# XinMing0411/AC-VAE

Measured on AMD Instinct MI355X. Metric: train-step captions/s (and audio-sec/s) at B=32, 1/2/4/8 MI355X, higher is better.
Workload: dtype f32

## Files before the change

### acvae_amd/build.py

```python
import os
import subprocess
import sys
from concurrent.futures import ThreadPoolExecutor

HERE = os.path.dirname(os.path.abspath(__file__))
CSRC = os.path.join(HERE, "csrc")
LIB = os.path.join(HERE, "libacvae_hip.so")
HIPCC = os.environ.get("HIPCC", "/opt/rocm/bin/hipcc")
FLAGS = ["-O3", "--offload-arch=gfx950", "-fPIC", "-std=c++17", "-Wall", "-Wno-unused-function",
         "-ffp-contract=off"]
if os.environ.get("ACVAE_EXACT_TANH") == "1":
    FLAGS.append("-DACVAE_EXACT_TANH")


def sources():
    return sorted(f for f in os.listdir(CSRC) if f.endswith(".hip"))


def _newer(a, b):
    return (not os.path.exists(b)) or os.path.getmtime(a) > os.path.getmtime(b)


def parse_usage(text):
    import re
    out, name = {}, None
    for line in text.splitlines():
        m = re.search(r"Function Name: (\S+)", line)
        if m:
            name = m.group(1)
            out[name] = {}
            continue
        for key, pat in (("vgprs", r" VGPRs: (\d+)"), ("sgprs", r" SGPRs: (\d+)"), ("scratch", r"ScratchSize \[bytes/lane\]: (\d+)"),
                         ("occupancy", r"Occupancy \[waves/SIMD\]: (\d+)")):
            m = re.search(pat, line)
            if m and name:
                out[name][key] = int(m.group(1))
    return out


def resource_usage():
    usage = {}
    for s in sources():
        path = os.path.join(CSRC, s[:-4] + ".usage.txt")
        if os.path.exists(path):
            usage.update(parse_usage(open(path).read()))
    return usage


def build(force=False, verbose=False):
    hdrs = [os.path.join(CSRC, f) for f in os.listdir(CSRC) if f.endswith(".h")]
    hdrs.append(os.path.join(os.path.dirname(HERE), "include", "acvae_hip.h"))
    objs, jobs = [], []
    for s in sources():
        src = os.path.join(CSRC, s)
        obj = os.path.join(CSRC, s[:-4] + ".o")
        objs.append(obj)
        if force or _newer(src, obj) or any(_newer(h, obj) for h in hdrs) or not os.path.exists(obj[:-2] + ".usage.txt"):
            jobs.append([HIPCC, *FLAGS, "-Rpass-analysis=kernel-resource-usage", "-c", src, "-o", obj])

    def run(cmd):
        if verbose:
            print(" ".join(cmd), flush=True)
        r = subprocess.run(cmd, capture_output=True, text=True)
        if r.returncode != 0:
            raise RuntimeError("hipcc failed:\n" + " ".join(cmd) + "\n" + r.stdout + r.stderr)
        if "-c" in cmd:
            remarks = "\n".join(l for l in r.stderr.splitlines() if "kernel-resource-usage" in l)
            open(cmd[-1][:-2] + ".usage.txt", "w").write(remarks)
            import re as _re
            rest = "\n".join(l for l in r.stderr.splitlines() if "kernel-resource-usage" not in l and
                             not _re.match(r"^\s*(\d+)?\s*\|", l)).strip()
            if verbose:
                for k, u in sorted(parse_usage(remarks).items()):
                    if u.get("scratch", 0) or u.get("vgprs", 0) >= 200:
                        print(f"  {k[:90]}: {u.get('vgprs')} VGPRs, {u.get('scratch')} B/lane scratch, occupancy {u.get('occupancy')}")
                if rest:
                    print(rest)
        elif verbose and r.stderr.strip():
            print(r.stderr)

    with ThreadPoolExecutor(max_workers=min(6, max(1, len(jobs)))) as ex:
        list(ex.map(run, jobs))
    if jobs or not os.path.exists(LIB):
        run([HIPCC, "--offload-arch=gfx950", "-shared", "-fPIC", "-o", LIB, *objs])
    return LIB


if __name__ == "__main__":
    print(build(force="--force" in sys.argv, verbose=True))
```

### acvae_amd/csrc/conv.h

```cpp
#pragma once
#include <hip/hip_runtime.h>
#include <stdint.h>
#include "common.h"
#include "job_table.h"

struct DropoutSpec {
  float p;
  const uint8_t* mask;
  uint64_t seed;
  uint32_t site;
};

enum { UP_PLAIN = 0, UP_POOL = 1, UP_DROP = 2 };

namespace acvae {
int conv3x3_igemm(const float* X, const float* scale, const float* shift, const float* Wp, float* Y, float* partials,
                  int N, int H, int W, int Cin, int Cout, hipStream_t st);
int conv_partials_rows(int N, int H, int W);
int conv3x3_igemm_bf16(const bf16_t* X, const float* scale, const float* shift, const bf16_t* Wp, bf16_t* Y,
                       float* partials, int N, int H, int W, int Cin, int Cout, hipStream_t st);
long conv3x3_wgrad_bf16_slab_floats(int N, int H, int W, int Cin, int Cout);
int conv3x3_wgrad_bf16_splits(int N, int H, int W, int Cin, int Cout);
int conv3x3_wgrad_bf16_launch(const bf16_t* dY, const bf16_t* X, const float* scale, const float* shift, float* slab, int N,
                              int H, int W, int Cin, int Cout, hipStream_t st);
int wgrad_reduce(const float* slab, int nsplit, float* dW_oihw, int Cout, int Cin, hipStream_t st);
long conv3x3_wgrad_slab_floats(int N, int H, int W, int Cin, int Cout);
int conv3x3_wgrad(const float* dY, const float* X, const float* scale, const float* shift, float* dW_oihw, float* slab,
                  int N, int H, int W, int Cin, int Cout, hipStream_t st);
bool conv3x3_wino_ok(int H, int W, int Cin, int Cout);
long conv3x3_wino_weight_floats(int Cin, int Cout);
int conv_wino_partials_rows(int N, int H, int W);
int conv3x3_wino_weights(const float* W_oihw, float* U, int Cout, int Cin, bool dgrad, hipStream_t st);
struct WinoWeightsJob { const float* W; float* U; int Cout, Cin, dgrad; };
using WinoWeightsBatch = RangeTable<WinoWeightsJob, 32>;
int conv3x3_wino_weights_batch(WinoWeightsBatch& b, hipStream_t st);
struct WinoBnReduce { const float* Y; const float* scale; const float* shift; const float* mean; const float* invstd; };
int conv3x3_wino(const float* X, const float* scale, const float* shift, const float* U, float* Y, float* partials, int N,
                 int H, int W, int Cin, int Cout, hipStream_t st, const WinoBnReduce* red = nullptr);
bool conv3x3_wino_wgrad_ok(int H, int W, int Cin, int Cout);
long conv3x3_wino_wgrad_slab_floats(int N, int H, int W, int Cin, int Cout);
int conv3x3_wino_wgrad(const float* dY, const float* X, const float* scale, const float* shift, float* dW_oihw, float* slab,
                       int N, int H, int W, int Cin, int Cout, hipStream_t st);
template <class T>
int repack_weights(const float* W_oihw, T* Wf, T* Wd, int Cout, int Cin, hipStream_t st);
struct RepackJob { const float* W; void* dst; int Cout, Cin, dgrad; };
using RepackBatch = RangeTable<RepackJob, 32>;
template <class T>
int repack_weights_batch(RepackBatch& b, hipStream_t st);
inline int conv3x3_igemm(const bf16_t* X, const float* scale, const float* shift, const bf16_t* Wp, bf16_t* Y,
                         float* partials, int N, int H, int W, int Cin, int Cout, hipStream_t st) {
  return conv3x3_igemm_bf16(X, scale, shift, Wp, Y, partials, N, H, W, Cin, Cout, st);
}
inline int conv3x3_wgrad(const bf16_t* dY, const bf16_t* X, const float* scale, const float* shift, float* dW_oihw,
                         float* slab, int N, int H, int W, int Cin, int Cout, hipStream_t st) {
  int r = conv3x3_wgrad_bf16_launch(dY, X, scale, shift, slab, N, H, W, Cin, Cout, st);
  if (r != 0) return r;
  return wgrad_reduce(slab, conv3x3_wgrad_bf16_splits(N, H, W, Cin, Cout), dW_oihw, Cout, Cin, st);
}
template <class T>
inline long conv3x3_wgrad_slab_floats_t(int N, int H, int W, int Cin, int Cout) {
  return sizeof(T) == 2 ? conv3x3_wgrad_bf16_slab_floats(N, H, W, Cin, Cout) : conv3x3_wgrad_slab_floats(N, H, W, Cin, Cout);
}
int bn0_stats(const float* x, float* partials, long rows, int F, int* nparts, hipStream_t st);
int bn0_partials_rows(long rows);
int bn_finalize(const float* partials, int P, int C, double count, const float* gamma, const float* beta,
                float* running_mean, float* running_var, int64_t* nbt, int training, float* scale, float* shift,
                float* mean, float* invstd, double* dpart, hipStream_t st);
long colsum_scratch_doubles(int width);
int colsum_tickets_reset(double* dpart, hipStream_t st);
long colsum_ticket_words();
int colsum2(const float* x, int P, int width, double* dpart, float* out, float* out2, int split, hipStream_t st);
struct ColsumJob { const float* x; int P, width; float* out; float* out_b; int R; long d0; };
using ColsumBatch = RangeTable<ColsumJob, 6, int>;
int colsum_batch(ColsumBatch& b, double* dpart, long dpart_doubles, hipStream_t st);
int conv1_first_blocks(int N, int T);
template <class TY>
int conv1_first_fwd(const float* x, const float* scale0, const float* shift0, const float* W1, TY* Y,
                    float* partials, int N, int T, int F, hipStream_t st);
template <class TY>
int conv1_first_bwd(const float* x, const float* scale0, const float* shift0, const float* mean0, const float* invstd0,
                    const float* W1, const TY* dY, float* dw_part, float* bn_part, float* dW1, float* dgamma0,
                    float* dbeta0, double* dpart, int N, int T, int F, hipStream_t st);
template <class T>
int bn_relu_pool(const T* Y, const float* scale, const float* shift, T* P, int N, int H, int W, int C,
                 DropoutSpec drop, hipStream_t st, bool pool = true);
int bn_bwd_blocks(int N, int H, int W, int C);
template <class T>
int bn_bwd(const T* Y, const T* dO, int upstream, const float* scale, const float* shift, const float* mean,
           const float* invstd, float* partials, float* sum_g, float* sum_gy, T* dY, double* dpart, int N, int H,
           int W, int C, DropoutSpec drop, hipStream_t st, bool batch_stats = true, int ready_rows = 0);
template <class T>
int relu_mask(const T* Y, const float* scale, const float* shift, uint8_t* out, int N, int H, int W, int C, hipStream_t st);
template <class T>
int freq_mean(const T* P, float* out, long rows, int Fp, int C, hipStream_t st);
template <class T>
int freq_mean_bwd(const float* dae, T* dP, long rows, int Fp, int C, hipStream_t st);
int time_pool(const float* ae, float* out, int N, int S, int C, DropoutSpec drop, hipStream_t st);
int relu_dropout(float* x, int total, DropoutSpec drop, hipStream_t st);
}

int acvae_gemm_nt_dual(const float* A1, int64_t lda1, const float* B1, int64_t ldb1, int K1, const float* A2,
                       int64_t lda2, const float* B2, int64_t ldb2, int K2, const float* bias, float* C, int64_t ldc,
                       int M, int N, int accumulate, hipStream_t st, float* skws = nullptr);
int acvae_gemm_nt_pair(const float* A0, int64_t lda0, const float* B0, int64_t ldb0, int K0, const float* bias0, float* C0,
                       int64_t ldc0, int N0, int acc0, const float* A1, int64_t lda1, const float* B1, int64_t ldb1, int K1,
                       const float* bias1, float* C1, int64_t ldc1, int N1, int acc1, int M, hipStream_t st);
constexpr int TN_TICKETS = 256;
int acvae_gemm_tn_fused(const float* A, int64_t lda, const float* B, int64_t ldb, float* C, int64_t ldc, int M, int N, int K,
                        int accumulate, float* ws, int64_t ws_bytes, hipStream_t st);
long acvae_skinny_ws_floats();
long acvae_skinny_ticket_words();
int acvae_skinny_ws_reset(float* ws, hipStream_t st);
struct TransposeJob { const float* in; long ld_in; float* out; long ld_out; int rows, cols; };
using TransposeBatch = acvae::RangeTable<TransposeJob, 12, int>;
int acvae_transpose_batch(TransposeBatch& b, hipStream_t st);
```

### acvae_amd/csrc/decoder.hip

```cpp
#include <cstdlib>
#include "common.h"
#include "conv.h"
#include "rnn.h"
#include "decode_persist.h"
#include "../../include/acvae_hip.h"

namespace {

struct Bump {
  long off = 0;
  long take(long n) { const long o = off; off = (off + n + 63) & ~63L; return o; }
};

struct Ctx {
  hipStream_t s;
  float* skws;
  operator hipStream_t() const { return s; }
};
inline int gemm(const float* A, long lda, const float* B, long ldb, const float* bias, float* C, long ldc, int M, int N,
                int K, int acc, const Ctx& st) {
  return acvae_gemm_nt_dual(A, lda, B, ldb, K, nullptr, 0, nullptr, 0, 0, bias, C, ldc, M, N, acc, st.s, st.skws);
}
inline int gemm2(const float* A1, long lda1, const float* B1, long ldb1, int K1, const float* A2, long lda2,
                 const float* B2, long ldb2, int K2, const float* bias, float* C, long ldc, int M, int N, int acc,
                 const Ctx& st) {
  if (M <= 64)
    return acvae_gemm_nt_dual(A1, lda1, B1, ldb1, K1, A2, lda2, B2, ldb2, K2, bias, C, ldc, M, N, acc, st.s, st.skws);
  ACVAE_TRY(acvae_gemm_nt_dual(A1, lda1, B1, ldb1, K1, nullptr, 0, nullptr, 0, 0, bias, C, ldc, M, N, acc, st.s, st.skws));
  return acvae_gemm_nt_dual(A2, lda2, B2, ldb2, K2, nullptr, 0, nullptr, 0, 0, nullptr, C, ldc, M, N, 1, st.s, st.skws);
}
struct TnWs { float* p; long bytes; };
inline int gemm_tn(const float* A, long lda, const float* B, long ldb, float* C, long ldc, int M, int N, int K, TnWs ws,
                   hipStream_t st) {
  return acvae_gemm_tn_fused(A, lda, B, ldb, C, ldc, M, N, K, 0, ws.p, ws.bytes, st);
}
inline void zb_skinny(acvae::ZeroBatch& zb, float* skws) { zb.add(skws, acvae_skinny_ticket_words()); }
inline void zb_colsum(acvae::ZeroBatch& zb, double* dpart) { zb.add(dpart, acvae::colsum_ticket_words()); }
inline void zb_tn(acvae::ZeroBatch& zb, TnWs ws) { zb.add(ws.p, TN_TICKETS); }
inline int transp(const float* in, long ld_in, float* out, long ld_out, int rows, int cols, hipStream_t st) {
  return acvae_transpose(in, ld_in, out, ld_out, rows, cols, st);
}
inline int zero(float* p, long n, hipStream_t st) {
  return hipMemsetAsync(p, 0, (size_t)n * sizeof(float), st) == hipSuccess ? ACVAE_OK : (int)hipGetLastError();
}
struct Fork {
  hipStream_t main_s, aux;
  bool on() const { return aux != main_s; }
  static int edge(hipStream_t from, hipStream_t to) {
    constexpr int RING = 64;
    struct Ring { hipEvent_t ev[RING]; int next; int dev; };
    static thread_local Ring ring = {{}, 0, -1};
    int dev = -1;
    if (hipGetDevice(&dev) != hipSuccess) return (int)hipGetLastError();
    if (dev != ring.dev) {
      for (int i = 0; i < RING; ++i) ring.ev[i] = nullptr;
      ring.next = 0; ring.dev = dev;
    }
    hipEvent_t& e = ring.ev[ring.next];
    ring.next = (ring.next + 1) % RING;
    if (!e && hipEventCreateWithFlags(&e, hipEventDisableTiming) != hipSuccess) return (int)hipGetLastError();
    hipError_t r = hipEventRecord(e, from);
    if (r == hipSuccess) r = hipStreamWaitEvent(to, e, 0);
    return r == hipSuccess ? ACVAE_OK : (int)r;
  }
  int begin() const { return on() ? edge(main_s, aux) : ACVAE_OK; }
  int join() const { return on() ? edge(aux, main_s) : ACVAE_OK; }
};
inline long tn_ws_floats(int M, int N, int K) { return acvae_gemm_tn_workspace_bytes(M, N, K) / 4 + 64 + TN_TICKETS; }

enum {
  TP_DEC_EMB, TP_DEC_WIH, TP_DEC_WHH, TP_DEC_BIH, TP_DEC_BHH, TP_DEC_CLS_W, TP_DEC_CLS_B, TP_DEC_ATT_V, TP_DEC_ATT_W,
  TP_DEC_ATT_B, TP_Q_EMB, TP_Q_WIH, TP_Q_WHH, TP_Q_BIH, TP_Q_BHH, TP_Q_WIH_R, TP_Q_WHH_R, TP_Q_BIH_R, TP_Q_BHH_R,
  TP_Q_TML_W, TP_Q_TML_B, TP_P_EMB, TP_P_ATT_V, TP_P_ATT_W, TP_P_ATT_B, TP_P_WIH, TP_P_WHH, TP_P_BIH, TP_P_BHH,
  TP_P_ML_W, TP_P_ML_B, TP_MLO_W, TP_MLO_B, TP_LN_W, TP_LN_B, TP_COUNT
};
static_assert(TP_COUNT == ACVAE_TEXT_NPARAMS, "text parameter table out of sync with the header");

struct PostLayout {
  long words, x, hidden, save_f, save_r, hprev_f, hprev_r, argmax, saved_total;
  long gi_f, gi_r, gh, hf, ml, dml, dhid, dgi_f, dgi_r, dgh_f, dgh_r, dh_a, dh_b, dx, wt, wt2, wt_ih0, wt_ih1, wt_ml, pq_hbuf, pq_cnt, tn, dpart, skws,
       scratch_total;
  long tn_floats, dpart_doubles;
};
int post_layout(int N, int Tc, int E, int Hq, int V, PostLayout& L) {
  if (N <= 0 || Tc <= 0 || E <= 0 || Hq <= 0 || V <= 0) return ACVAE_EINVAL;
  const long R = (long)N * Tc;
  Bump s;
  L.words = s.take(R * 2);
  L.x = s.take(R * E);
  L.hidden = s.take(R * 2 * Hq);
  L.save_f = s.take(R * 4 * Hq); L.save_r = s.take(R * 4 * Hq);
  L.hprev_f = s.take(R * Hq); L.hprev_r = s.take(R * Hq);
  L.argmax = s.take((long)N * 2 * Hq);
  L.saved_total = s.off;
  Bump c;
  L.gi_f = c.take(R * 3 * Hq); L.gi_r = c.take(R * 3 * Hq);
  L.gh = c.take((long)N * 3 * Hq); L.hf = c.take((long)N * Hq);
  L.ml = c.take(R * 2 * E); L.dml = c.take(R * 2 * E); L.dhid = c.take(R * 2 * Hq);
  L.dgi_f = c.take(R * 3 * Hq); L.dgi_r = c.take(R * 3 * Hq); L.dgh_f = c.take(R * 3 * Hq); L.dgh_r = c.take(R * 3 * Hq);
  L.dh_a = c.take((long)N * Hq); L.dh_b = c.take((long)N * Hq);
  L.dx = c.take(R * E);
  long wt = (long)2 * E * 2 * Hq;
  if ((long)3 * Hq * Hq > wt) wt = (long)3 * Hq * Hq;
  if ((long)3 * Hq * E > wt) wt = (long)3 * Hq * E;
  L.wt = c.take(wt);
  L.wt2 = c.take((long)3 * Hq * Hq);
  L.wt_ih0 = c.take((long)3 * Hq * E); L.wt_ih1 = c.take((long)3 * Hq * E); L.wt_ml = c.take((long)2 * E * 2 * Hq);
  L.pq_hbuf = c.take((long)4 * N * Hq);
  L.pq_cnt = c.take(acvae::posterior_persist_counter_words(Tc));
  long tn = tn_ws_floats(2 * E, 2 * Hq, (int)R);
  long t2 = tn_ws_floats(3 * Hq, E, (int)R); if (t2 > tn) tn = t2;
  t2 = tn_ws_floats(3 * Hq, Hq, (int)R); if (t2 > tn) tn = t2;
  L.tn_floats = tn;
  L.tn = c.take(tn);
  L.dpart_doubles = 4 * acvae::colsum_scratch_doubles(2 * E > 3 * Hq ? 2 * E : 3 * Hq);
  L.dpart = c.take(2 * L.dpart_doubles);
  L.skws = c.take(acvae_skinny_ws_floats());
  L.scratch_total = c.off;
  return ACVAE_OK;
}

struct DecLayout {
  long words, mem, encproj_d, encproj_p, qd, qp, attw_p, rnn_d, rnn_p, gru_save, hprev_d, lstm_save, c_all, hp_all,
      hpprev, lse, pool_arg, pool_hid, unfinished, saved_total;
  long wt_cls, wt_dih, wt_dhh, wt_datt, wt_pih, wt_phh, wt_pml, wt_patt, wt_mlo;
  long skws, skws_p, gi_d, gh_d, gates_p, ml, h0, pd_cnt, attfws_d, attfws_p, attfws_bytes, scratch_fwd;
  long wt_ln;
  long d_out, dgi, dgh, dqd, dencproj, dvpart, dctx, dh_a, dh_b, dgates, dml_all, dml, dhp_a, dhp_b, dc_a, dc_b, dlz_a, pd_part,
      dlz_b, drnn, dz_dec, dqp, dmem, dhid, words_c, tn, dpart, attws, pd_cnt_b, pd_dqd, scratch_bwd;
  long dencproj_p, dvpart_p, dmem_p, drnn_p, tn_p, dpart_p, attws_p;
  long attws_bytes;
  long tn_floats, tn_p_floats, dpart_doubles;
};
int dec_layout(int N, int Tc, int S, int E, int H, int A, int V, int Eenc, DecLayout& L) {
  if (N <= 0 || Tc <= 0 || S <= 0 || E <= 0 || H <= 0 || A <= 0 || V <= 1 || Eenc <= 0) return ACVAE_EINVAL;
  const long R = (long)N * Tc;
  const int Hp = E;
  Bump s;
  L.words = s.take(R * 2);
  L.mem = s.take((long)N * S * E);
  L.encproj_d = s.take((long)N * S * A); L.encproj_p = s.take((long)N * S * E);
  L.qd = s.take(R * A); L.qp = s.take(R * E); L.attw_p = s.take(R * S);
  L.rnn_d = s.take(R * 3 * E); L.rnn_p = s.take(R * 3 * E);
  L.gru_save = s.take(R * 4 * H); L.hprev_d = s.take(R * H);
  L.lstm_save = s.take(R * 5 * Hp); L.c_all = s.take(R * Hp); L.hp_all = s.take(R * Hp); L.hpprev = s.take(R * Hp);
  L.lse = s.take(R); L.pool_arg = s.take((long)N * H); L.pool_hid = s.take((long)N * H);
  L.unfinished = s.take(N);
  L.wt_cls = s.take((long)H * V + 64); L.wt_dih = s.take((long)3 * E * 3 * H); L.wt_dhh = s.take((long)H * 3 * H);
  L.wt_datt = s.take((long)(E + H) * A); L.wt_pih = s.take((long)3 * E * 4 * Hp); L.wt_phh = s.take((long)Hp * 4 * Hp);
  L.wt_pml = s.take((long)Hp * 2 * E); L.wt_patt = s.take((long)2 * E * E); L.wt_mlo = s.take((long)H * 2 * E);
  L.saved_total = s.off;
  Bump f;
  L.skws = f.take(acvae_skinny_ws_floats());
  L.skws_p = f.take(acvae_skinny_ws_floats());
  L.gi_d = f.take(R * 3 * H); L.gh_d = f.take((long)N * 3 * H); L.gates_p = f.take(R * 4 * Hp);
  L.ml = f.take((long)N * 2 * E); L.h0 = f.take((long)N * (H > Hp ? H : Hp));
  L.pd_cnt = f.take(acvae::decode_persist_counter_words(Tc));
  L.attfws_bytes = acvae_attn_fwd_workspace_bytes(N, 1, S, A, E);
  { const long w2 = acvae_attn_fwd_workspace_bytes(N, 1, S, E, E); if (w2 > L.attfws_bytes) L.attfws_bytes = w2; }
  L.attfws_d = f.take(L.attfws_bytes / 4 + 64); L.attfws_p = f.take(L.attfws_bytes / 4 + 64);
  L.scratch_fwd = f.off;
  Bump b;
  b.take(acvae_skinny_ws_floats());
  b.take(acvae_skinny_ws_floats());
  L.wt_ln = b.take((long)Eenc * E);
  L.d_out = b.take(R * H); L.dgi = b.take(R * 3 * H); L.dgh = b.take(R * 3 * H); L.dqd = b.take(R * A);
  L.dencproj = b.take((long)N * S * (A > E ? A : E));
  L.dvpart = b.take((long)3 * N * (A > E ? A : E));
  L.dctx = b.take((long)N * E); L.dh_a = b.take((long)N * H); L.dh_b = b.take((long)N * H);
  L.dgates = b.take(R * 4 * Hp); L.dml_all = b.take(R * 2 * E); L.dml = b.take((long)N * 2 * E);
  L.dhp_a = b.take((long)N * Hp); L.dhp_b = b.take((long)N * Hp); L.dc_a = b.take((long)N * Hp);
  L.dc_b = b.take((long)N * Hp); L.dlz_a = b.take((long)N * E); L.dlz_b = b.take((long)N * E);
  L.drnn = b.take(R * 3 * E); L.dz_dec = b.take(R * E); L.dqp = b.take(R * E);
  L.dmem = b.take((long)N * S * E); L.dhid = b.take((long)N * H); L.words_c = b.take(R * 2);
  long tn = 0;
  auto mx = [&](int M, int Nn, int K) { const long t = tn_ws_floats(M, Nn, K); if (t > tn) tn = t; };
  mx(V, H, (int)R); mx(3 * H, 3 * E, (int)R); mx(3 * H, H, (int)R); mx(A, H, (int)R); mx(A, E, N * S); mx(E, E, N * S);
  mx(4 * Hp, 3 * E, (int)R); mx(4 * Hp, Hp, (int)R); mx(2 * E, Hp, (int)R); mx(E, E, (int)R); mx(2 * E, H, N);
  mx(E, Eenc, N * S);
  L.tn_floats = tn;
  L.tn = b.take(tn);
  {
    int w = V; if (4 * Hp > w) w = 4 * Hp; if (3 * H > w) w = 3 * H; if (2 * E > w) w = 2 * E; if (A > w) w = A;
    L.dpart_doubles = acvae::colsum_scratch_doubles(w);
    L.dpart = b.take(2 * L.dpart_doubles);
  }
  L.attws_bytes = acvae_attn_bwd_workspace_bytes(N, Tc, S, A > E ? A : E);
  L.attws = b.take(L.attws_bytes / 4 + 64);
  L.attws_p = b.take(L.attws_bytes / 4 + 64);
  L.dencproj_p = b.take((long)N * S * E); L.dvpart_p = b.take((long)N * E); L.dmem_p = b.take((long)N * S * E);
  L.drnn_p = b.take(R * 3 * E);
  L.tn_p_floats = L.tn_floats;
  L.tn_p = b.take(L.tn_p_floats);
  {
    int w = V; if (4 * Hp > w) w = 4 * Hp; if (3 * H > w) w = 3 * H; if (2 * E > w) w = 2 * E; if (A > w) w = A;
    L.dpart_p = b.take(2 * acvae::colsum_scratch_doubles(w));
  }
  L.pd_cnt_b = b.take(acvae::decode_persist_bwd_counter_words(Tc));
  L.pd_part = b.take(acvae::decode_persist_bwd_part_floats(N, E, H));
  L.pd_dqd = b.take(S > 64 && S <= 192 ? (long)acvae::decode_persist_bwd_rc_splits(S) * R * A : 0);
  L.scratch_bwd = b.off;
  return ACVAE_OK;
}

}

extern "C" int64_t acvae_posterior_saved_bytes(int N, int Tc, int E, int Hq, int V) {
  PostLayout L;
  return post_layout(N, Tc, E, Hq, V, L) == ACVAE_OK ? L.saved_total * 4 : -1;
}
extern "C" int64_t acvae_posterior_scratch_bytes(int N, int Tc, int E, int Hq, int V) {
  PostLayout L;
  return post_layout(N, Tc, E, Hq, V, L) == ACVAE_OK ? L.scratch_total * 4 : -1;
}

extern "C" int acvae_posterior_fwd(const void* const* params, const int64_t* caps, int64_t ld_caps, const int64_t* lens1,
                                   const float* eps_q, float* q_means, float* q_logs, float* q_z, float* q_means_utt,
                                   void* saved_v, int64_t saved_bytes, void* scratch_v, int64_t scratch_bytes, int N,
                                   int Tc, int E, int Hq, int V, void* stream, int flags) {
  PostLayout L;
  ACVAE_TRY(post_layout(N, Tc, E, Hq, V, L));
  if (!params || !caps || !lens1 || !eps_q || !q_means || !q_logs || !q_z || !q_means_utt || !saved_v || !scratch_v)
    return ACVAE_EINVAL;
  if (saved_bytes < L.saved_total * 4 || scratch_bytes < L.scratch_total * 4) return ACVAE_EWORKSPACE;
  float* sv = (float*)saved_v;
  float* sc = (float*)scratch_v;
  Ctx st{(hipStream_t)stream, sc + L.skws};
  const bool persist_q = !(flags & ACVAE_FLAG_NO_PERSIST) && acvae::posterior_persist_ok(N, Tc, Hq);
  {
    acvae::ZeroBatch zb;
    zb_skinny(zb, st.skws);
    if (persist_q) {
      zb.add(sc + L.pq_cnt, acvae::posterior_persist_counter_words(Tc));
      zb.add(sc + L.pq_hbuf, (long)4 * N * Hq);
      flags |= ACVAE_FLAG_INT_CNT_ZEROED;
    }
    ACVAE_TRY(acvae::zero_batch(zb, st.s));
  }
  auto P = [&](int i) { return (const float*)params[i]; };
  const int R = N * Tc;
  int64_t* words = (int64_t*)(sv + L.words);
  float* X = sv + L.x;
  float* hid = sv + L.hidden;
  ACVAE_TRY(acvae::gather_words(caps, ld_caps, 1, words, N, Tc, st));
  ACVAE_TRY(acvae::embed_gather(words, 1, P(TP_Q_EMB), V, X, E, R, E, st));
  if (persist_q) {
    PqParams pq;
    for (int dir = 0; dir < 2; ++dir) {
      const int o = dir * 4;
      float* gi = sc + (dir ? L.gi_r : L.gi_f);
      ACVAE_TRY(gemm(X, E, P(TP_Q_WIH + o), E, P(TP_Q_BIH + o), gi, 3 * Hq, R, 3 * Hq, E, 0, st));
      pq.w_hh[dir] = P(TP_Q_WHH + o); pq.b_hh[dir] = P(TP_Q_BHH + o); pq.gi[dir] = gi;
      pq.save[dir] = sv + (dir ? L.save_r : L.save_f);
      pq.hprev[dir] = sv + (dir ? L.hprev_r : L.hprev_f);
    }
    pq.lens1 = lens1; pq.hid = hid; pq.hbuf = sc + L.pq_hbuf; pq.cnt = (unsigned*)(sc + L.pq_cnt);
    pq.N = N; pq.Tc = Tc; pq.Hq = Hq;
    ACVAE_TRY(acvae::posterior_persist_fwd(pq, st.s, flags));
  } else
  for (int dir = 0; dir < 2; ++dir) {
    const int o = dir * 4;
    float* gi = sc + (dir ? L.gi_r : L.gi_f);
    float* save = sv + (dir ? L.save_r : L.save_f);
    float* hprev = sv + (dir ? L.hprev_r : L.hprev_f);
    float* h = sc + L.hf;
    float* gh = sc + L.gh;
    ACVAE_TRY(gemm(X, E, P(TP_Q_WIH + o), E, P(TP_Q_BIH + o), gi, 3 * Hq, R, 3 * Hq, E, 0, st));
    ACVAE_TRY(acvae::copy_rows(h, Hq, nullptr, 0, N, Hq, st));
    for (int k = 0; k < Tc; ++k) {
      const int t = dir ? Tc - 1 - k : k;
      ACVAE_TRY(gemm(h, Hq, P(TP_Q_WHH + o), Hq, P(TP_Q_BHH + o), gh, 3 * Hq, N, 3 * Hq, Hq, 0, st));
      ACVAE_TRY(acvae::gru_fwd(gi + (long)t * 3 * Hq, (long)Tc * 3 * Hq, gh, 3 * Hq, h, Hq, h, Hq,
                               hid + (long)t * 2 * Hq + dir * Hq, (long)Tc * 2 * Hq, save + (long)t * 4 * Hq,
                               (long)Tc * 4 * Hq, hprev + (long)t * Hq, (long)Tc * Hq, lens1, t, N, Hq, st));
    }
  }
  float* ml = sc + L.ml;
  ACVAE_TRY(gemm(hid, 2 * Hq, P(TP_Q_TML_W), 2 * Hq, P(TP_Q_TML_B), ml, 2 * E, R, 2 * E, 2 * Hq, 0, st));
  ACVAE_TRY(acvae_reparam_fwd(ml, 2 * E, eps_q, E, q_means, q_logs, q_z, E, nullptr, 0, R, E, st));
  ACVAE_TRY(acvae::pool_fwd(hid, (long)Tc * 2 * Hq, 2 * Hq, lens1, q_means_utt, (int*)(sv + L.argmax), N, Tc, 2 * Hq, st));
  return ACVAE_OK;
}

extern "C" int acvae_posterior_bwd(const void* const* params, void* const* grads, const int64_t* lens1,
                                   const float* eps_q, const float* q_logs, const float* d_q_means,
                                   const float* d_q_logs, const float* d_q_z, const float* d_q_means_utt, void* saved_v,
                                   int64_t saved_bytes, void* scratch_v, int64_t scratch_bytes, int N, int Tc, int E,
                                   int Hq, int V, void* stream, int flags) {
  PostLayout L;
  ACVAE_TRY(post_layout(N, Tc, E, Hq, V, L));
  if (!params || !grads || !lens1 || !eps_q || !q_logs || !saved_v || !scratch_v) return ACVAE_EINVAL;
  if (saved_bytes < L.saved_total * 4 || scratch_bytes < L.scratch_total * 4) return ACVAE_EWORKSPACE;
  float* sv = (float*)saved_v;
  float* sc = (float*)scratch_v;
  Ctx st{(hipStream_t)stream, sc + L.skws};
  auto P = [&](int i) { return (const float*)params[i]; };
  auto G = [&](int i) { return (float*)grads[i]; };
  const int R = N * Tc;
  TnWs tn{sc + L.tn, L.tn_floats * 4};
  double* dpart = (double*)(sc + L.dpart);
  const bool persist = !(flags & ACVAE_FLAG_NO_PERSIST) && acvae::posterior_persist_ok(N, Tc, Hq);
  {
    acvae::ZeroBatch zb;
    zb_skinny(zb, st.skws); zb_colsum(zb, dpart); zb_tn(zb, tn);
    if (persist) { zb.add(sc + L.pq_cnt, acvae::posterior_persist_counter_words(Tc)); flags |= ACVAE_FLAG_INT_CNT_ZEROED; }
    zb.add(G(TP_Q_EMB), (long)V * E);
    ACVAE_TRY(acvae::zero_batch(zb, st.s));
  }
  const int64_t* words = (const int64_t*)(sv + L.words);
  float* X = sv + L.x;
  float* hid = sv + L.hidden;
  float* dml = sc + L.dml;
  float* dhid = sc + L.dhid;
  float* wt = sc + L.wt;
  float* wt_ml = sc + L.wt_ml;
  float* wt_ih[2] = {sc + L.wt_ih0, sc + L.wt_ih1};
  {
    TransposeBatch tb;
    tb.add({P(TP_Q_TML_W), 2 * Hq, wt_ml, 2 * E, 2 * E, 2 * Hq});
    for (int dir = 0; dir < 2; ++dir) {
      tb.add({P(TP_Q_WIH + dir * 4), E, wt_ih[dir], 3 * Hq, 3 * Hq, E});
      if (persist) tb.add({P(TP_Q_WHH + dir * 4), Hq, dir ? sc + L.wt2 : wt, 3 * Hq, 3 * Hq, Hq});
    }
    ACVAE_TRY(acvae_transpose_batch(tb, st.s));
  }
  ACVAE_TRY(acvae_reparam_bwd(d_q_z, E, d_q_means, d_q_logs, E, q_logs, E, eps_q, E, dml, 2 * E, R, E, st));
  ACVAE_TRY(gemm(dml, 2 * E, wt_ml, 2 * E, nullptr, dhid, 2 * Hq, R, 2 * Hq, 2 * E, 0, st));
  if (d_q_means_utt)
    ACVAE_TRY(acvae::pool_bwd(d_q_means_utt, lens1, (const int*)(sv + L.argmax), dhid, (long)Tc * 2 * Hq, 2 * Hq, 1, N,
                              Tc, 2 * Hq, st));
  ACVAE_TRY(gemm_tn(dml, 2 * E, hid, 2 * Hq, G(TP_Q_TML_W), 2 * Hq, 2 * E, 2 * Hq, R, tn, st));
  acvae::ColsumBatch cb;
  cb.add({dml, R, 2 * E, G(TP_Q_TML_B)});
  float* dx = sc + L.dx;
  if (persist) {
    PqbParams pb;
    for (int dir = 0; dir < 2; ++dir) {
      pb.wt[dir] = dir ? sc + L.wt2 : wt;
      pb.save[dir] = sv + (dir ? L.save_r : L.save_f);
      pb.hprev[dir] = sv + (dir ? L.hprev_r : L.hprev_f);
      pb.dgi[dir] = sc + (dir ? L.dgi_r : L.dgi_f);
      pb.dgh[dir] = sc + (dir ? L.dgh_r : L.dgh_f);
    }
    pb.dhid = dhid; pb.lens1 = lens1; pb.cnt = (unsigned*)(sc + L.pq_cnt);
    pb.N = N; pb.Tc = Tc; pb.Hq = Hq;
    ACVAE_TRY(acvae::posterior_persist_bwd(pb, st.s, flags));
  }
  for (int dir = 0; dir < 2; ++dir) {
    const int o = dir * 4;
    float* save = sv + (dir ? L.save_r : L.save_f);
    float* hprev = sv + (dir ? L.hprev_r : L.hprev_f);
    float* dgi = sc + (dir ? L.dgi_r : L.dgi_f);
    float* dgh = sc + (dir ? L.dgh_r : L.dgh_f);
    float* dh = sc + L.dh_a;
    float* dh2 = sc + L.dh_b;
    if (!persist) {
      ACVAE_TRY(transp(P(TP_Q_WHH + o), Hq, wt, 3 * Hq, 3 * Hq, Hq, st));
      ACVAE_TRY(acvae::copy_rows(dh, Hq, nullptr, 0, N, Hq, st));
      for (int k = 0; k < Tc; ++k) {
        const int t = dir ? k : Tc - 1 - k;
        ACVAE_TRY(acvae::gru_bwd(dh, Hq, dhid + (long)t * 2 * Hq + dir * Hq, (long)Tc * 2 * Hq, save + (long)t * 4 * Hq,
                                 (long)Tc * 4 * Hq, hprev + (long)t * Hq, (long)Tc * Hq, dgi + (long)t * 3 * Hq,
                                 (long)Tc * 3 * Hq, dgh + (long)t * 3 * Hq, (long)Tc * 3 * Hq, dh2, Hq, lens1, t, N, Hq,
                                 st));
        ACVAE_TRY(gemm(dgh + (long)t * 3 * Hq, (long)Tc * 3 * Hq, wt, 3 * Hq, nullptr, dh2, Hq, N, Hq, 3 * Hq, 1, st));
        float* tmp = dh; dh = dh2; dh2 = tmp;
      }
    }
    ACVAE_TRY(gemm_tn(dgi, 3 * Hq, X, E, G(TP_Q_WIH + o), E, 3 * Hq, E, R, tn, st));
    cb.add({dgi, R, 3 * Hq, G(TP_Q_BIH + o)});
    ACVAE_TRY(gemm_tn(dgh, 3 * Hq, hprev, Hq, G(TP_Q_WHH + o), Hq, 3 * Hq, Hq, R, tn, st));
    cb.add({dgh, R, 3 * Hq, G(TP_Q_BHH + o)});
    ACVAE_TRY(gemm(dgi, 3 * Hq, wt_ih[dir], 3 * Hq, nullptr, dx, E, R, E, 3 * Hq, dir, st));
  }
  ACVAE_TRY(acvae::colsum_batch(cb, dpart, L.dpart_doubles, st));
  ACVAE_TRY(acvae::embed_scatter(words, dx, E, G(TP_Q_EMB), V, R, E, st));
  return ACVAE_OK;
}

extern "C" int64_t acvae_decode_saved_bytes(int N, int Tc, int S, int E, int H, int A, int V, int Eenc) {
  DecLayout L;
  return dec_layout(N, Tc, S, E, H, A, V, Eenc, L) == ACVAE_OK ? L.saved_total * 4 : -1;
}
extern "C" int64_t acvae_decode_scratch_bytes(int N, int Tc, int S, int E, int H, int A, int V, int Eenc) {
  DecLayout L;
  if (dec_layout(N, Tc, S, E, H, A, V, Eenc, L) != ACVAE_OK) return -1;
  return (L.scratch_fwd > L.scratch_bwd ? L.scratch_fwd : L.scratch_bwd) * 4;
}

extern "C" int acvae_decode_fwd(const void* const* params, const float* mem_in, const int64_t* mem_lens,
                                const int64_t* caps, int64_t ld_caps, const int64_t* lens1, const float* q_z,
                                const float* eps_p, const int* ss_flags_host, const int* dis_flags_host, float* logits,
                                float* outputs, int64_t* seqs, float* sampled_logprobs, float* attn_w, float* p_means,
                                float* p_logs, float* p_z, float* p_means_utt, float* h_final, float* hp_final,
                                float* cp_final, void* saved_v, int64_t saved_bytes, void* scratch_v,
                                int64_t scratch_bytes, int N, int Tc, int S, int E, int H, int A, int V, int Eenc,
                                int start_idx, int end_idx, void* stream, void* aux_stream, int flags) {
  return acvae_decode_fwd_sampled(params, mem_in, mem_lens, caps, ld_caps, lens1, q_z, eps_p, ss_flags_host,
                                  dis_flags_host, logits, outputs, seqs, sampled_logprobs, attn_w, p_means, p_logs, p_z,
                                  p_means_utt, h_final, hp_final, cp_final, saved_v, saved_bytes, scratch_v,
                                  scratch_bytes, N, Tc, S, E, H, A, V, Eenc, start_idx, end_idx, stream, aux_stream,
                                  ACVAE_SAMPLE_GREEDY, 1.f, nullptr, nullptr, 0.f, flags);
}

extern "C" int acvae_decode_fwd_sampled(const void* const* params, const float* mem_in, const int64_t* mem_lens,
                                        const int64_t* caps, int64_t ld_caps, const int64_t* lens1, const float* q_z,
                                        const float* eps_p, const int* ss_flags_host, const int* dis_flags_host,
                                        float* logits, float* outputs, int64_t* seqs, float* sampled_logprobs,
                                        float* attn_w, float* p_means, float* p_logs, float* p_z, float* p_means_utt,
                                        float* h_final, float* hp_final, float* cp_final, void* saved_v,
                                        int64_t saved_bytes, void* scratch_v, int64_t scratch_bytes, int N, int Tc, int S,
                                        int E, int H, int A, int V, int Eenc, int start_idx, int end_idx, void* stream,
                                        void* aux_stream, int sample_method, float temp, const float* sample_noise,
                                        const uint8_t* emb_keep, float emb_drop_p, int flags) {
  if (emb_keep && !(emb_drop_p > 0.f && emb_drop_p <= 1.f)) return ACVAE_EINVAL;
  if (sample_method != ACVAE_SAMPLE_GREEDY &&
      ((sample_method != ACVAE_SAMPLE_GUMBEL && sample_method != ACVAE_SAMPLE_MULTINOMIAL) || !sample_noise ||
       !(temp > 0.f)))
    return ACVAE_EINVAL;
  DecLayout L;
  ACVAE_TRY(dec_layout(N, Tc, S, E, H, A, V, Eenc, L));
  if (!params || !mem_in || !mem_lens || !eps_p || !logits || !outputs || !seqs || !sampled_logprobs || !attn_w ||
      !p_means || !p_logs || !p_z || !saved_v || !scratch_v)
    return ACVAE_EINVAL;
  const bool train = caps != nullptr;
  if (train && (!lens1 || !q_z || !ss_flags_host || !dis_flags_host || !p_means_utt)) return ACVAE_EINVAL;
  if (train && H != E) return ACVAE_EUNSUPPORTED;
  if (saved_bytes < L.saved_total * 4 || scratch_bytes < L.scratch_fwd * 4) return ACVAE_EWORKSPACE;
  float* sv = (float*)saved_v;
  float* sc = (float*)scratch_v;
  auto P = [&](int i) { return (const float*)params[i]; };
  const int R = N * Tc, Hp = E;
  const bool has_ln = Eenc != E || params[TP_LN_W] != nullptr;
  bool teacher = train, prior_feeds_decoder = !train;
  if (train)
    for (int t = 0; t < Tc; ++t) {
      teacher = teacher && ss_flags_host[t] != 0;
      prior_feeds_decoder = prior_feeds_decoder || dis_flags_host[t] != 0;
    }
  Ctx st{(hipStream_t)stream, sc + L.skws};
  const Fork fork{st.s, (aux_stream && teacher) ? (hipStream_t)aux_stream : st.s};
  Ctx sp{fork.aux, sc + L.skws_p};
  const bool persist_fwd = teacher && !prior_feeds_decoder && !(flags & ACVAE_FLAG_NO_PERSIST) && H == E &&
                           acvae::decode_persist_ok(N, Tc, S, E, H, A);
  const bool attws_ready = !persist_fwd && L.attfws_bytes > 0;
  {
    acvae::ZeroBatch zb;
    zb_skinny(zb, st.skws); zb_skinny(zb, sp.skws);
    if (attws_ready) { zb.add(sc + L.attfws_d, 256); zb.add(sc + L.attfws_p, 256); }
    if (persist_fwd) { zb.add(sc + L.pd_cnt, acvae::decode_persist_counter_words(Tc)); flags |= ACVAE_FLAG_INT_CNT_ZEROED; }
    ACVAE_TRY(acvae::zero_batch(zb, st.s));
  }

  int64_t* words = (int64_t*)(sv + L.words);
  const float* mem = has_ln ? sv + L.mem : mem_in;
  float* encproj_d = sv + L.encproj_d;
  float* encproj_p = sv + L.encproj_p;
  float* qd = sv + L.qd;
  float* qp = sv + L.qp;
  float* attw_p = sv + L.attw_p;
  float* rnn_d = sv + L.rnn_d;
  float* rnn_p = sv + L.rnn_p;
  float* gi_d = sc + L.gi_d;
  float* gh_d = sc + L.gh_d;
  float* gates_p = sc + L.gates_p;
  float* ml = sc + L.ml;
  float* zeros = sc + L.h0;
  uint8_t* unfinished = (uint8_t*)(sv + L.unfinished);
  const long ld3E = (long)Tc * 3 * E;

  if (has_ln) ACVAE_TRY(gemm(mem_in, Eenc, P(TP_LN_W), Eenc, P(TP_LN_B), sv + L.mem, E, N * S, E, Eenc, 0, st));
  auto encproj_prior = [&](const Ctx& c) -> int {
    return gemm(mem, E, P(TP_P_ATT_W) + E, 2 * E, P(TP_P_ATT_B), encproj_p, E, N * S, E, E, 0, c);
  };
  auto encproj_dec = [&]() -> int {
    ACVAE_TRY(gemm(mem, E, P(TP_DEC_ATT_W) + H, E + H, P(TP_DEC_ATT_B), encproj_d, A, N * S, A, E, 0, st));
    return acvae::copy_rows(zeros, H > Hp ? H : Hp, nullptr, 0, N, H > Hp ? H : Hp, st);
  };

  auto rows_of = [&](int cnt) { return cnt == Tc ? R : N; };
  auto ldof = [&](int cnt, long C) { return cnt == Tc ? C : (long)Tc * C; };
  auto prior_pre = [&](int t0, int cnt) -> int {
    const int M = rows_of(cnt);
    ACVAE_TRY(acvae::embed_gather(words + t0, cnt == Tc ? 1 : Tc, P(TP_P_EMB), V, rnn_p + (long)t0 * 3 * E,
                                  ldof(cnt, 3 * E), M, E, sp));
    ACVAE_TRY(gemm(rnn_p + (long)t0 * 3 * E, ldof(cnt, 3 * E), P(TP_P_ATT_W), 2 * E, nullptr, qp + (long)t0 * E,
                   ldof(cnt, E), M, E, E, 0, sp));
    ACVAE_TRY(acvae_attn_fwd(qp + (long)t0 * E, (long)Tc * E, E, encproj_p, mem, mem_lens, P(TP_P_ATT_V),
                             rnn_p + (long)t0 * 3 * E + E, ld3E, 3 * E, attw_p + (long)t0 * S, (long)Tc * S, S, N, cnt, S,
                             E, E, (cnt == 1 && attws_ready) ? sc + L.attfws_p : nullptr, L.attfws_bytes, sp, flags));
    ACVAE_TRY(gemm(rnn_p + (long)t0 * 3 * E, ldof(cnt, 3 * E), P(TP_P_WIH), 3 * E, P(TP_P_BIH),
                   gates_p + (long)t0 * 4 * Hp, ldof(cnt, 4 * Hp), M, 4 * Hp, 2 * E, 0, sp));
    return ACVAE_OK;
  };
  float* hp_all = sv + L.hp_all;
  float* c_all = sv + L.c_all;
  float* hpprev = sv + L.hpprev;
  float* lstm_save = sv + L.lstm_save;
  auto prior_step = [&](int t) -> int {
    const float* hprev = t ? hp_all + (long)(t - 1) * Hp : zeros;
    const long ldh = t ? (long)Tc * Hp : Hp;
    const float* cprev = t ? c_all + (long)(t - 1) * Hp : nullptr;
    if (t == 0) ACVAE_TRY(acvae::copy_rows(rnn_p + 2 * E, ld3E, nullptr, 0, N, E, sp));
    ACVAE_TRY(gemm2(rnn_p + (long)t * 3 * E + 2 * E, ld3E, P(TP_P_WIH) + 2 * E, 3 * E, E, hprev, ldh, P(TP_P_WHH), Hp,
                    Hp, P(TP_P_BHH), gates_p + (long)t * 4 * Hp, (long)Tc * 4 * Hp, N, 4 * Hp, 1, sp));
    ACVAE_TRY(acvae::lstm_fwd(gates_p + (long)t * 4 * Hp, (long)Tc * 4 * Hp, cprev, (long)Tc * Hp,
                              hp_all + (long)t * Hp, (long)Tc * Hp, c_all + (long)t * Hp, (long)Tc * Hp,
                              lstm_save + (long)t * 5 * Hp, (long)Tc * 5 * Hp, N, Hp, sp));
    ACVAE_TRY(gemm(hp_all + (long)t * Hp, (long)Tc * Hp, P(TP_P_ML_W), Hp, P(TP_P_ML_B), ml, 2 * E, N, 2 * E, Hp, 0, sp));
    float* z2 = (t + 1 < Tc) ? rnn_p + (long)(t + 1) * 3 * E + 2 * E : nullptr;
    ACVAE_TRY(acvae_reparam_fwd(ml, 2 * E, eps_p + (long)t * N * E, E, p_means + (long)t * E, p_logs + (long)t * E,
                                p_z + (long)t * E, (long)Tc * E, z2, ld3E, N, E, sp));
    return ACVAE_OK;
  };
  auto dec_pre = [&](int t0, int cnt) -> int {
    const int M = rows_of(cnt);
    ACVAE_TRY(acvae::embed_gather(words + t0, cnt == Tc ? 1 : Tc, P(TP_DEC_EMB), V, rnn_d + (long)t0 * 3 * E,
                                  ldof(cnt, 3 * E), M, E, st));
    if (emb_keep)
      ACVAE_TRY(acvae::dropout_rows(rnn_d + (long)t0 * 3 * E, ld3E, 3 * E, emb_keep + (long)t0 * N * E, E, (long)N * E,
                                    emb_drop_p < 1.f ? 1.f / (1.f - emb_drop_p) : 0.f, N, cnt, E, st));
    if (cnt == Tc && train && !prior_feeds_decoder) {
      ACVAE_TRY(acvae::copy_rows(rnn_d + 2 * E, 3 * E, q_z, E, R, E, st));
    } else {
      for (int t = t0; t < t0 + cnt; ++t) {
        const float* zsrc = (train && !dis_flags_host[t]) ? q_z : p_z;
        ACVAE_TRY(acvae::copy_rows(rnn_d + (long)t * 3 * E + 2 * E, ld3E, zsrc + (long)t * E, (long)Tc * E, N, E, st));
      }
    }
    ACVAE_TRY(gemm2(rnn_d + (long)t0 * 3 * E, ldof(cnt, 3 * E), P(TP_DEC_WIH), 3 * E, E,
                    rnn_d + (long)t0 * 3 * E + 2 * E, ldof(cnt, 3 * E), P(TP_DEC_WIH) + 2 * E, 3 * E, E, P(TP_DEC_BIH),
                    gi_d + (long)t0 * 3 * H, ldof(cnt, 3 * H), M, 3 * H, 0, st));
    return ACVAE_OK;
  };
  float* gru_save = sv + L.gru_save;
  float* hprev_d = sv + L.hprev_d;
  static const bool pair_env = !(getenv("ACVAE_SKINNY_PAIR") && atoi(getenv("ACVAE_SKINNY_PAIR")) == 0);
  const bool pair_ok = pair_env && N <= 64;
  auto dec_step = [&](int t) -> int {
    const float* hprev = t ? outputs + (long)(t - 1) * H : zeros;
    const long ldh = t ? (long)Tc * H : H;
    if (pair_ok) {
      ACVAE_TRY(acvae_gemm_nt_pair(hprev, ldh, P(TP_DEC_ATT_W), E + H, H, nullptr, qd + (long)t * A, (long)Tc * A, A, 0,
                                   hprev, ldh, P(TP_DEC_WHH), H, H, P(TP_DEC_BHH), gh_d, 3 * H, 3 * H, 0, N, st));
    } else {
      ACVAE_TRY(gemm(hprev, ldh, P(TP_DEC_ATT_W), E + H, nullptr, qd + (long)t * A, (long)Tc * A, N, A, H, 0, st));
      ACVAE_TRY(gemm(hprev, ldh, P(TP_DEC_WHH), H, P(TP_DEC_BHH), gh_d, 3 * H, N, 3 * H, H, 0, st));
    }
    ACVAE_TRY(acvae_attn_fwd(qd + (long)t * A, (long)Tc * A, A, encproj_d, mem, mem_lens, P(TP_DEC_ATT_V),
                             rnn_d + (long)t * 3 * E + E, ld3E, 3 * E, attn_w + (long)t * S, (long)Tc * S, S, N, 1, S, A,
                             E, attws_ready ? sc + L.attfws_d : nullptr, L.attfws_bytes, st, flags));
    ACVAE_TRY(gemm(rnn_d + (long)t * 3 * E + E, ld3E, P(TP_DEC_WIH) + E, 3 * E, nullptr, gi_d + (long)t * 3 * H,
                   (long)Tc * 3 * H, N, 3 * H, E, 1, st));
    ACVAE_TRY(acvae::gru_fwd(gi_d + (long)t * 3 * H, (long)Tc * 3 * H, gh_d, 3 * H, hprev, ldh, outputs + (long)t * H,
                             (long)Tc * H, nullptr, 0, gru_save + (long)t * 4 * H, (long)Tc * 4 * H,
                             hprev_d + (long)t * H, (long)Tc * H, nullptr, t, N, H, st));
    return ACVAE_OK;
  };
  auto transposes = [&](hipStream_t ts) -> int {
    if (!train) return ACVAE_OK;
    TransposeBatch tb;
    tb.add({P(TP_DEC_CLS_W), H, sv + L.wt_cls, V, V, H});
    tb.add({P(TP_DEC_WIH), 3 * E, sv + L.wt_dih, 3 * H, 3 * H, 3 * E});
    tb.add({P(TP_DEC_WHH), H, sv + L.wt_dhh, 3 * H, 3 * H, H});
    tb.add({P(TP_DEC_ATT_W), E + H, sv + L.wt_datt, A, A, E + H});
    tb.add({P(TP_P_WIH), 3 * E, sv + L.wt_pih, 4 * Hp, 4 * Hp, 3 * E});
    tb.add({P(TP_P_WHH), Hp, sv + L.wt_phh, 4 * Hp, 4 * Hp, Hp});
    tb.add({P(TP_P_ML_W), Hp, sv + L.wt_pml, 2 * E, 2 * E, Hp});
    tb.add({P(TP_P_ATT_W), 2 * E, sv + L.wt_patt, E, E, 2 * E});
    tb.add({P(TP_MLO_W), H, sv + L.wt_mlo, 2 * E, 2 * E, H});
    return acvae_transpose_batch(tb, ts);
  };
  float* lse = sv + L.lse;
  auto classify = [&](int t0, int cnt) -> int {
    const int M = rows_of(cnt);
    ACVAE_TRY(gemm(outputs + (long)t0 * H, ldof(cnt, H), P(TP_DEC_CLS_W), H, P(TP_DEC_CLS_B), logits + (long)t0 * V,
                   ldof(cnt, V), M, V, H, 0, st));
    ACVAE_TRY(acvae_row_logsoftmax_argmax(logits + (long)t0 * V, (long)Tc * V, V, seqs + t0, sampled_logprobs + t0,
                                          lse + t0, Tc, 1, N, cnt, V, st));
    if (sample_method != ACVAE_SAMPLE_GREEDY)
      ACVAE_TRY(acvae_sample_next_word(logits + (long)t0 * V, (long)Tc * V, V, sample_noise + (long)t0 * N * V, V,
                                       (long)N * V, sample_method, temp, seqs + t0, sampled_logprobs + t0, Tc, 1, N, cnt,
                                       V, st));
    return ACVAE_OK;
  };

  if (teacher) {
    ACVAE_TRY(acvae::gather_words(caps, ld_caps, 1, words, N, Tc, st));
    ACVAE_TRY(fork.begin());
    ACVAE_TRY(encproj_prior(sp));
    ACVAE_TRY(encproj_dec());
    ACVAE_TRY(prior_pre(0, Tc));
    if (prior_feeds_decoder) {
      for (int t = 0; t < Tc; ++t) ACVAE_TRY(prior_step(t));
      ACVAE_TRY(fork.join());
      ACVAE_TRY(dec_pre(0, Tc));
      for (int t = 0; t < Tc; ++t) ACVAE_TRY(dec_step(t));
    } else if (persist_fwd) {
      ACVAE_TRY(dec_pre(0, Tc));
      ACVAE_TRY(acvae::copy_rows(rnn_p + 2 * E, ld3E, nullptr, 0, N, E, sp));
      ACVAE_TRY(fork.join());
      PdParams pd{};
      pd.w_att = P(TP_DEC_ATT_W); pd.w_hh = P(TP_DEC_WHH); pd.b_hh = P(TP_DEC_BHH); pd.w_ih = P(TP_DEC_WIH);
      pd.att_v = P(TP_DEC_ATT_V);
      pd.pw_ih = P(TP_P_WIH); pd.pw_hh = P(TP_P_WHH); pd.pb_hh = P(TP_P_BHH); pd.w_ml = P(TP_P_ML_W); pd.b_ml = P(TP_P_ML_B);
      pd.encproj = encproj_d; pd.mem = mem; pd.mem_lens = mem_lens; pd.gi = gi_d; pd.gates_p = gates_p;
      pd.eps_p = eps_p; pd.zeros = zeros;
      pd.qd = qd; pd.gh = gh_d; pd.rnn_d = rnn_d; pd.attn_w = attn_w; pd.outputs = outputs; pd.gru_save = sv + L.gru_save;
      pd.hprev_d = sv + L.hprev_d; pd.rnn_p = rnn_p; pd.hp_all = sv + L.hp_all; pd.c_all = sv + L.c_all;
      pd.lstm_save = sv + L.lstm_save; pd.p_means = p_means; pd.p_logs = p_logs; pd.p_z = p_z;
      pd.cnt = (unsigned*)(sc + L.pd_cnt);
      pd.N = N; pd.Tc = Tc; pd.S = S; pd.E = E; pd.H = H; pd.A = A;
      ACVAE_TRY(acvae::decode_persist_fwd(pd, st.s, flags));
    } else {
      ACVAE_TRY(dec_pre(0, Tc));
      for (int t = 0; t < Tc; ++t) {
        ACVAE_TRY(prior_step(t));
        ACVAE_TRY(dec_step(t));
      }
    }
    ACVAE_TRY(transposes(sp.s));
    ACVAE_TRY(classify(0, Tc));
    ACVAE_TRY(fork.join());
  } else {
    ACVAE_TRY(encproj_dec());
    ACVAE_TRY(encproj_prior(st));
    for (int t = 0; t < Tc; ++t) {
      ACVAE_TRY(acvae::select_word(caps, ld_caps, seqs, Tc, words, Tc, t, train && ss_flags_host[t], start_idx, N, st));
      ACVAE_TRY(prior_pre(t, 1));
      ACVAE_TRY(prior_step(t));
      ACVAE_TRY(dec_pre(t, 1));
      ACVAE_TRY(dec_step(t));
      ACVAE_TRY(classify(t, 1));
      if (!train) ACVAE_TRY(acvae::finish_rows(seqs, Tc, unfinished, t, end_idx, N, st));
    }
    ACVAE_TRY(transposes(st.s));
  }
  {
    acvae::CopyRowsBatch cb;
    cb.add({hpprev, (long)Tc * Hp, nullptr, 0, N, Hp});
    if (Tc > 1) cb.add({hpprev + Hp, (long)Tc * Hp, hp_all, (long)Tc * Hp, N, (Tc - 1) * Hp});
    if (h_final) cb.add({h_final, H, outputs + (long)(Tc - 1) * H, (long)Tc * H, N, H});
    if (hp_final) cb.add({hp_final, Hp, hp_all + (long)(Tc - 1) * Hp, (long)Tc * Hp, N, Hp});
    if (cp_final) cb.add({cp_final, Hp, c_all + (long)(Tc - 1) * Hp, (long)Tc * Hp, N, Hp});
    ACVAE_TRY(acvae::copy_rows_batch(cb, st));
  }
  if (train) {
    float* hidp = sv + L.pool_hid;
    ACVAE_TRY(acvae::pool_fwd(outputs, (long)Tc * H, H, lens1, hidp, (int*)(sv + L.pool_arg), N, Tc, H, st));
    ACVAE_TRY(gemm(hidp, H, P(TP_MLO_W), H, P(TP_MLO_B), p_means_utt, 2 * E, N, 2 * E, H, 0, st));
  }
  return ACVAE_OK;
}

extern "C" int acvae_decode_bwd_defers(const int* dis_flags_host, int Tc, void* stream, void* aux_stream, int flags) {
  if (!(flags & ACVAE_FLAG_DEFER_PARAM_GRADS) || !aux_stream || aux_stream == stream || !dis_flags_host) return 0;
  for (int t = 0; t < Tc; ++t)
    if (dis_flags_host[t] != 0) return 0;
  return 1;
}

extern "C" int acvae_decode_bwd(const void* const* params, void* const* grads, const float* mem_in,
                                const int64_t* mem_lens, const int64_t* lens1, const float* eps_p,
                                const int* dis_flags_host, const float* outputs, const float* attn_w,
                                const float* p_logs, const float* d_logits, const float* d_outputs_ext,
                                const float* d_p_means, const float* d_p_logs, const float* d_p_z,
                                const float* d_p_means_utt, float* d_mem_in, float* d_q_z, void* saved_v,
                                int64_t saved_bytes, void* scratch_v, int64_t scratch_bytes, int N, int Tc, int S, int E,
                                int H, int A, int V, int Eenc, void* stream, void* aux_stream, const uint8_t* emb_keep,
                                float emb_drop_p, int flags) {
  if (emb_keep && !(emb_drop_p > 0.f && emb_drop_p <= 1.f)) return ACVAE_EINVAL;
  DecLayout L;
  ACVAE_TRY(dec_layout(N, Tc, S, E, H, A, V, Eenc, L));
  if (!params || !grads || !mem_in || !mem_lens || !lens1 || !eps_p || !dis_flags_host || !outputs || !attn_w ||
      !p_logs || !d_mem_in || !d_q_z || !saved_v || !scratch_v)
    return ACVAE_EINVAL;
  if (saved_bytes < L.saved_total * 4 || scratch_bytes < L.scratch_bwd * 4) return ACVAE_EWORKSPACE;
  float* sv = (float*)saved_v;
  float* sc = (float*)scratch_v;
  bool prior_feeds_decoder = false;
  for (int t = 0; t < Tc; ++t) prior_feeds_decoder = prior_feeds_decoder || dis_flags_host[t] != 0;
  Ctx st{(hipStream_t)stream, sc + L.skws};
  const Fork fork{st.s, aux_stream ? (hipStream_t)aux_stream : st.s};
  Ctx sp{fork.aux, sc + L.skws_p};
  auto P = [&](int i) { return (const float*)params[i]; };
  auto G = [&](int i) { return (float*)grads[i]; };
  const int R = N * Tc, Hp = E;
  const bool defer = acvae_decode_bwd_defers(dis_flags_host, Tc, stream, aux_stream, flags) != 0;
  const bool has_ln = Eenc != E || params[TP_LN_W] != nullptr;
  TnWs tn{sc + L.tn, L.tn_floats * 4};
  TnWs tn_p{sc + L.tn_p, L.tn_p_floats * 4};
  double* dpart = (double*)(sc + L.dpart);
  double* dpart_p = (double*)(sc + L.dpart_p);
  const bool persist_bwd = !prior_feeds_decoder && !(flags & ACVAE_FLAG_NO_PERSIST) && acvae::decode_persist_bwd_ok(N, Tc, S, E, H, A);
  {
    acvae::ZeroBatch zb;
    zb_skinny(zb, st.skws); zb_skinny(zb, sp.skws); zb_colsum(zb, dpart); zb_colsum(zb, dpart_p); zb_tn(zb, tn); zb_tn(zb, tn_p);
    if (persist_bwd) {
      zb.add(sc + L.pd_cnt_b, acvae::decode_persist_bwd_counter_words(Tc));
      zb.add(sc + L.dmem_p, (long)N * S * E);
      flags |= ACVAE_FLAG_INT_CNT_ZEROED;
    }
    zb.add(G(TP_DEC_EMB), (long)V * E); zb.add(G(TP_P_EMB), (long)V * E);
    ACVAE_TRY(acvae::zero_batch(zb, st.s));
  }
  const int64_t* words = (const int64_t*)(sv + L.words);
  const float* mem = has_ln ? sv + L.mem : mem_in;
  float* rnn_d = sv + L.rnn_d;
  float* rnn_p = sv + L.rnn_p;

  float *wt_cls = sv + L.wt_cls, *wt_dih = sv + L.wt_dih, *wt_dhh = sv + L.wt_dhh, *wt_datt = sv + L.wt_datt;
  float *wt_pih = sv + L.wt_pih, *wt_phh = sv + L.wt_phh, *wt_pml = sv + L.wt_pml, *wt_patt = sv + L.wt_patt;
  float *wt_mlo = sv + L.wt_mlo, *wt_ln = sc + L.wt_ln;
  int64_t* words_c = (int64_t*)(sc + L.words_c);
  ACVAE_TRY(acvae::gather_words(words, Tc, 1, words_c, N, Tc, st));
  ACVAE_TRY(fork.begin());

  float* d_out = sc + L.d_out;
  if (d_outputs_ext) ACVAE_TRY(acvae::copy_rows(d_out, H, d_outputs_ext, H, R, H, st));
  else ACVAE_TRY(zero(d_out, (long)R * H, st));
  if (d_p_means_utt) {
    float* dhid = sc + L.dhid;
    ACVAE_TRY(gemm(d_p_means_utt, 2 * E, wt_mlo, 2 * E, nullptr, dhid, H, N, H, 2 * E, 0, st));
    ACVAE_TRY(acvae::pool_bwd(dhid, lens1, (const int*)(sv + L.pool_arg), d_out, (long)Tc * H, H, 1, N, Tc, H, st));
  }
  if (d_logits) ACVAE_TRY(gemm(d_logits, V, wt_cls, V, nullptr, d_out, H, R, H, V, 1, st));
  auto heads_params = [&](const Ctx& c, TnWs ws, double* dp) -> int {
    acvae::ColsumBatch cb;
    if (d_p_means_utt) {
      ACVAE_TRY(gemm_tn(d_p_means_utt, 2 * E, sv + L.pool_hid, H, G(TP_MLO_W), H, 2 * E, H, N, ws, c));
      cb.add({d_p_means_utt, N, 2 * E, G(TP_MLO_B)});
    } else {
      ACVAE_TRY(zero(G(TP_MLO_W), (long)2 * E * H, c));
      ACVAE_TRY(zero(G(TP_MLO_B), 2 * E, c));
    }
    if (d_logits) {
      ACVAE_TRY(gemm_tn(d_logits, V, outputs, H, G(TP_DEC_CLS_W), H, V, H, R, ws, c));
      cb.add({d_logits, R, V, G(TP_DEC_CLS_B)});
    } else {
      ACVAE_TRY(zero(G(TP_DEC_CLS_W), (long)V * H, c));
      ACVAE_TRY(zero(G(TP_DEC_CLS_B), V, c));
    }
    return acvae::colsum_batch(cb, dp, L.dpart_doubles, c);
  };
  static const bool heads_aux = !(getenv("ACVAE_HEADS_AUX") && atoi(getenv("ACVAE_HEADS_AUX")) == 0);
  const bool heads_on_aux = heads_aux && fork.on();
  if (heads_on_aux) {
    ACVAE_TRY(heads_params(sp, tn_p, dpart_p));
  } else if (!defer) {
    ACVAE_TRY(heads_params(st, tn, dpart));
  }

  float* dgi = sc + L.dgi;
  float* dgh = sc + L.dgh;
  float* dqd = sc + L.dqd;
  float* dencproj = sc + L.dencproj;
  float* dvpart = sc + L.dvpart;
  float* dctx = sc + L.dctx;
  float* dmem = sc + L.dmem;
  float* dh = sc + L.dh_a;
  float* dh2 = sc + L.dh_b;
  const float* gru_save = sv + L.gru_save;
  const float* hprev_d = sv + L.hprev_d;
  const float* qd = sv + L.qd;
  auto dec_begin = [&]() -> int {
    ACVAE_TRY(zero(dencproj, (long)N * S * A, st));
    ACVAE_TRY(zero(dvpart, (long)N * A, st));
    ACVAE_TRY(zero(dmem, (long)N * S * E, st));
    ACVAE_TRY(zero(dh, (long)N * H, st));
    return ACVAE_OK;
  };
  float* drnn = sc + L.drnn;
  float* dz_dec = sc + L.dz_dec;
  int dv_rows = N;
  auto dec_bptt = [&](int t) -> int {
    ACVAE_TRY(acvae::gru_bwd(dh, H, d_out + (long)t * H, (long)Tc * H, gru_save + (long)t * 4 * H, (long)Tc * 4 * H,
                             hprev_d + (long)t * H, (long)Tc * H, dgi + (long)t * 3 * H, (long)Tc * 3 * H,
                             dgh + (long)t * 3 * H, (long)Tc * 3 * H, dh2, H, nullptr, t, N, H, st));
    ACVAE_TRY(gemm(dgi + (long)t * 3 * H, (long)Tc * 3 * H, wt_dih + (long)E * 3 * H, 3 * H, nullptr, dctx, E, N, E,
                   3 * H, 0, st));
    ACVAE_TRY(acvae_attn_bwd(dctx, E, 0, qd + (long)t * A, (long)Tc * A, A, sv + L.encproj_d, mem, mem_lens,
                             P(TP_DEC_ATT_V), attn_w + (long)t * S, (long)Tc * S, S, dqd + (long)t * A, (long)Tc * A, A,
                             dencproj, dmem, dvpart, sc + L.attws, L.attws_bytes, N, 1, S, A, E, st));
    ACVAE_TRY(gemm2(dgh + (long)t * 3 * H, (long)Tc * 3 * H, wt_dhh, 3 * H, 3 * H, dqd + (long)t * A, (long)Tc * A,
                    wt_datt, A, A, nullptr, dh2, H, N, H, 1, st));
    float* tmp = dh; dh = dh2; dh2 = tmp;
    return ACVAE_OK;
  };
  auto dec_memgrad = [&]() -> int {
    return gemm(dencproj, A, wt_datt + (long)H * A, A, nullptr, dmem, E, N * S, E, A, 1, st);
  };
  auto dec_dz = [&](const Ctx& c) -> int {
    ACVAE_TRY(gemm(dgi, 3 * H, wt_dih + (long)2 * E * 3 * H, 3 * H, nullptr, dz_dec, E, R, E, 3 * H, 0, c));
    if (!prior_feeds_decoder) {
      ACVAE_TRY(acvae::copy_rows(d_q_z, E, dz_dec, E, R, E, c));
    } else {
      for (int t = 0; t < Tc; ++t)
        ACVAE_TRY(acvae::copy_rows(d_q_z + (long)t * E, (long)Tc * E, dis_flags_host[t] ? nullptr : dz_dec + (long)t * E,
                                   (long)Tc * E, N, E, c));
    }
    return ACVAE_OK;
  };
  auto dec_params = [&](const Ctx& c, TnWs ws, double* dp, bool with_dz = true) -> int {
    ACVAE_TRY(gemm_tn(dgi, 3 * H, rnn_d, 3 * E, G(TP_DEC_WIH), 3 * E, 3 * H, 3 * E, R, ws, c));
    ACVAE_TRY(gemm_tn(dgh, 3 * H, hprev_d, H, G(TP_DEC_WHH), H, 3 * H, H, R, ws, c));
    {
      acvae::ColsumBatch cb;
      cb.add({dgi, R, 3 * H, G(TP_DEC_BIH)}); cb.add({dgh, R, 3 * H, G(TP_DEC_BHH)});
      cb.add({dencproj, N * S, A, G(TP_DEC_ATT_B)}); cb.add({dvpart, dv_rows, A, G(TP_DEC_ATT_V)});
      ACVAE_TRY(acvae::colsum_batch(cb, dp, L.dpart_doubles, c));
    }
    ACVAE_TRY(gemm_tn(dqd, A, hprev_d, H, G(TP_DEC_ATT_W), E + H, A, H, R, ws, c));
    ACVAE_TRY(gemm_tn(dencproj, A, mem, E, G(TP_DEC_ATT_W) + H, E + H, A, E, N * S, ws, c));
    ACVAE_TRY(gemm(dgi, 3 * H, wt_dih, 3 * H, nullptr, drnn, E, R, E, 3 * H, 0, c));
    if (emb_keep)
      ACVAE_TRY(acvae::dropout_rows(drnn, (long)Tc * E, E, emb_keep, E, (long)N * E, emb_drop_p < 1.f ? 1.f / (1.f - emb_drop_p) : 0.f, N, Tc, E, c));
    if (with_dz) ACVAE_TRY(dec_dz(c));
    ACVAE_TRY(acvae::embed_scatter(words_c, drnn, E, G(TP_DEC_EMB), V, R, E, c));
    return ACVAE_OK;
  };

  float* dgates = sc + L.dgates;
  float* dml_all = sc + L.dml_all;
  float* dhp = sc + L.dhp_a;
  float* dhp2 = sc + L.dhp_b;
  float* dc = sc + L.dc_a;
  float* dc2 = sc + L.dc_b;
  float* dlz = sc + L.dlz_a;
  float* dlz2 = sc + L.dlz_b;
  const float* lstm_save = sv + L.lstm_save;
  const float* c_all = sv + L.c_all;
  const float* hp_all = sv + L.hp_all;
  const float* hpprev = sv + L.hpprev;
  float* dpz = sc + L.dqp;
  float* drnn_p = sc + L.drnn_p;
  float* dencproj_p = sc + L.dencproj_p;
  float* dvpart_p = sc + L.dvpart_p;
  float* dmem_p = sc + L.dmem_p;
  auto prior_begin = [&]() -> int {
  for (int t = 0; t < Tc; ++t) {
    ACVAE_TRY(acvae::copy_rows(dpz + (long)t * E, (long)Tc * E, d_p_z ? d_p_z + (long)t * E : nullptr, (long)Tc * E, N, E,
                               sp));
    if (dis_flags_host[t])
      ACVAE_TRY(acvae::add_rows(dpz + (long)t * E, (long)Tc * E, dz_dec + (long)t * E, (long)Tc * E, N, E, sp));
  }
  ACVAE_TRY(zero(dmem_p, (long)N * S * E, sp));
  ACVAE_TRY(zero(dhp, (long)N * Hp, sp));
  ACVAE_TRY(zero(dc, (long)N * Hp, sp));
  ACVAE_TRY(zero(dlz, (long)N * E, sp));
    return ACVAE_OK;
  };
  auto prior_bptt = [&](int t) -> int {
    ACVAE_TRY(acvae::add_rows(dlz, E, dpz + (long)t * E, (long)Tc * E, N, E, sp));
    ACVAE_TRY(acvae_reparam_bwd(dlz, E, d_p_means ? d_p_means + (long)t * E : nullptr,
                                d_p_logs ? d_p_logs + (long)t * E : nullptr, (long)Tc * E, p_logs + (long)t * E,
                                (long)Tc * E, eps_p + (long)t * N * E, E, dml_all + (long)t * 2 * E, (long)Tc * 2 * E, N,
                                E, sp));
    ACVAE_TRY(gemm(dml_all + (long)t * 2 * E, (long)Tc * 2 * E, wt_pml, 2 * E, nullptr, dhp, Hp, N, Hp, 2 * E, 1, sp));
    ACVAE_TRY(acvae::lstm_bwd(dhp, Hp, dc, Hp, lstm_save + (long)t * 5 * Hp, (long)Tc * 5 * Hp,
                              t ? c_all + (long)(t - 1) * Hp : nullptr, (long)Tc * Hp, dgates + (long)t * 4 * Hp,
                              (long)Tc * 4 * Hp, dc2, Hp, N, Hp, sp));
    ACVAE_TRY(gemm(dgates + (long)t * 4 * Hp, (long)Tc * 4 * Hp, wt_phh, 4 * Hp, nullptr, dhp2, Hp, N, Hp, 4 * Hp, 0, sp));
    ACVAE_TRY(gemm(dgates + (long)t * 4 * Hp, (long)Tc * 4 * Hp, wt_pih + (long)2 * E * 4 * Hp, 4 * Hp, nullptr, dlz2, E,
                   N, E, 4 * Hp, 0, sp));
    float* tmp = dhp; dhp = dhp2; dhp2 = tmp;
    tmp = dc; dc = dc2; dc2 = tmp;
    tmp = dlz; dlz = dlz2; dlz2 = tmp;
    return ACVAE_OK;
  };
  float* dqp = sc + L.dqp;
  auto prior_memgrad = [&]() -> int {
    ACVAE_TRY(gemm(dgates, 4 * Hp, wt_pih, 4 * Hp, nullptr, drnn_p, 3 * E, R, 2 * E, 4 * Hp, 0, sp));
    ACVAE_TRY(zero(dencproj_p, (long)N * S * E, sp));
    ACVAE_TRY(zero(dvpart_p, (long)N * E, sp));
    ACVAE_TRY(acvae_attn_bwd(drnn_p + E, (long)Tc * 3 * E, 3 * E, sv + L.qp, (long)Tc * E, E, sv + L.encproj_p, mem,
                             mem_lens, P(TP_P_ATT_V), sv + L.attw_p, (long)Tc * S, S, dqp, (long)Tc * E, E, dencproj_p,
                             dmem_p, dvpart_p, sc + L.attws_p, L.attws_bytes, N, Tc, S, E, E, sp));
    return gemm(dencproj_p, E, wt_patt + (long)E * E, E, nullptr, dmem_p, E, N * S, E, E, 1, sp);
  };
  auto prior_params = [&]() -> int {
    ACVAE_TRY(gemm_tn(dml_all, 2 * E, hp_all, Hp, G(TP_P_ML_W), Hp, 2 * E, Hp, R, tn_p, sp));
    ACVAE_TRY(gemm_tn(dgates, 4 * Hp, rnn_p, 3 * E, G(TP_P_WIH), 3 * E, 4 * Hp, 3 * E, R, tn_p, sp));
    ACVAE_TRY(gemm_tn(dgates, 4 * Hp, hpprev, Hp, G(TP_P_WHH), Hp, 4 * Hp, Hp, R, tn_p, sp));
    {
      acvae::ColsumBatch cb;
      cb.add({dml_all, R, 2 * E, G(TP_P_ML_B)}); cb.add({dgates, R, 4 * Hp, G(TP_P_BIH), G(TP_P_BHH)});
      cb.add({dencproj_p, N * S, E, G(TP_P_ATT_B)}); cb.add({dvpart_p, N, E, G(TP_P_ATT_V)});
      ACVAE_TRY(acvae::colsum_batch(cb, dpart_p, L.dpart_doubles, sp));
    }
    ACVAE_TRY(gemm(dqp, E, wt_patt, E, nullptr, drnn_p, 3 * E, R, E, E, 1, sp));
    ACVAE_TRY(gemm_tn(dqp, E, rnn_p, 3 * E, G(TP_P_ATT_W), 2 * E, E, E, R, tn_p, sp));
    ACVAE_TRY(gemm_tn(dencproj_p, E, mem, E, G(TP_P_ATT_W) + E, 2 * E, E, E, N * S, tn_p, sp));
    return acvae::embed_scatter(words_c, drnn_p, 3 * E, G(TP_P_EMB), V, R, E, sp);
  };
  if (prior_feeds_decoder) {
    ACVAE_TRY(dec_begin());
    for (int t = Tc - 1; t >= 0; --t) ACVAE_TRY(dec_bptt(t));
    ACVAE_TRY(dec_memgrad());
    ACVAE_TRY(dec_params(st, tn, dpart));
    if (fork.on()) ACVAE_TRY(Fork::edge(st.s, sp.s));
    ACVAE_TRY(prior_begin());
    for (int t = Tc - 1; t >= 0; --t) ACVAE_TRY(prior_bptt(t));
    ACVAE_TRY(prior_memgrad());
    ACVAE_TRY(prior_params());
  } else if (persist_bwd) {
    PbParams pb{};
    pb.wt_dhh = wt_dhh; pb.wt_datt = wt_datt; pb.wt_dih = wt_dih; pb.wt_phh = wt_phh; pb.wt_pih = wt_pih; pb.wt_pml = wt_pml;
    pb.att_v = P(TP_DEC_ATT_V);
    pb.encproj = sv + L.encproj_d; pb.mem = mem; pb.qd = qd; pb.attn_w = attn_w; pb.gru_save = gru_save; pb.hprev_d = hprev_d;
    pb.lstm_save = lstm_save; pb.c_all = c_all; pb.p_logs = p_logs; pb.eps_p = eps_p; pb.mem_lens = mem_lens;
    pb.d_out = d_out; pb.d_p_z = d_p_z; pb.d_p_means = d_p_means; pb.d_p_logs = d_p_logs;
    pb.dgi = dgi; pb.dgh = dgh; pb.dqd = dqd; pb.dctx = drnn;
    pb.dencproj = dencproj; pb.dmem = dmem; pb.dvpart = dvpart; pb.dgates = dgates; pb.dml_all = dml_all; pb.dhp = dhp;
    pb.dctx_part = sc + L.pd_part; pb.dhp_part = pb.dctx_part + 4L * N * E; pb.dml_part = pb.dhp_part + 4L * N * E;
    pb.cnt = (unsigned*)(sc + L.pd_cnt_b);
    pb.dqd_part = sc + L.pd_dqd; pb.ctx = rnn_d + E;
    pb.N = N; pb.Tc = Tc; pb.S = S; pb.E = E; pb.H = H; pb.A = A;
    ACVAE_TRY(acvae::decode_persist_bwd(pb, st.s, flags));
    dv_rows = N * acvae::decode_persist_bwd_rc_splits(S);
    ACVAE_TRY(dec_memgrad());
    if (fork.on()) ACVAE_TRY(Fork::edge(st.s, sp.s));
    ACVAE_TRY(prior_memgrad());
    if (!defer) {
      ACVAE_TRY(dec_params(st, tn, dpart));
      ACVAE_TRY(prior_params());
    }
  } else {
    ACVAE_TRY(dec_begin());
    ACVAE_TRY(prior_begin());
    for (int t = Tc - 1; t >= 0; --t) {
      ACVAE_TRY(dec_bptt(t));
      ACVAE_TRY(prior_bptt(t));
    }
    ACVAE_TRY(dec_memgrad());
    ACVAE_TRY(prior_memgrad());
    if (!defer) {
      ACVAE_TRY(dec_params(st, tn, dpart));
      ACVAE_TRY(prior_params());
    }
  }
  ACVAE_TRY(fork.join());
  ACVAE_TRY(acvae::add_rows(dmem, E, dmem_p, E, N * S, E, st));
  if (has_ln) {
    ACVAE_TRY(transp(P(TP_LN_W), Eenc, wt_ln, E, E, Eenc, st));
    ACVAE_TRY(gemm(dmem, E, wt_ln, E, nullptr, d_mem_in, Eenc, N * S, Eenc, E, 0, st));
    ACVAE_TRY(gemm_tn(dmem, E, mem_in, Eenc, G(TP_LN_W), Eenc, E, Eenc, N * S, tn, st));
    ACVAE_TRY(acvae::colsum2(dmem, N * S, E, dpart, G(TP_LN_B), nullptr, 0, st));
  } else {
    ACVAE_TRY(acvae::copy_rows(d_mem_in, E, dmem, E, N * S, E, st));
  }
  if (defer) {
    ACVAE_TRY(dec_dz(st));
    ACVAE_TRY(Fork::edge(st.s, sp.s));
    if (!heads_on_aux) ACVAE_TRY(heads_params(sp, tn_p, dpart_p));
    ACVAE_TRY(dec_params(sp, tn_p, dpart_p, false));
    ACVAE_TRY(prior_params());
  }
  return ACVAE_OK;
}

extern "C" int acvae_caps_to_long(const float* caps, int64_t* out, int64_t n, void* stream) {
  if (!caps || !out || n <= 0) return ACVAE_EINVAL;
  return acvae::caps_to_long(caps, out, (long)n, (hipStream_t)stream);
}

namespace {
struct StepLayout { long skws, encproj, rnn, q, gates, gh, ml, words, attws, attws_bytes, total; };
int step_layout(int N, int S, int E, int H, int A, int V, StepLayout& L) {
  if (N <= 0 || S <= 0 || E <= 0 || H <= 0 || A <= 0 || V <= 1) return ACVAE_EINVAL;
  Bump b;
  L.skws = b.take(acvae_skinny_ws_floats());
  L.encproj = b.take((long)N * S * (A > E ? A : E));
  L.rnn = b.take((long)N * 3 * E);
  L.q = b.take((long)N * (A > E ? A : E));
  L.gates = b.take((long)N * 4 * E);
  L.gh = b.take((long)N * 3 * H);
  L.ml = b.take((long)N * 2 * E);
  L.words = b.take((long)N * 2);
  L.attws_bytes = acvae_attn_fwd_workspace_bytes(N, 1, S, A, E);
  const long w2 = acvae_attn_fwd_workspace_bytes(N, 1, S, E, E);
  if (w2 > L.attws_bytes) L.attws_bytes = w2;
  L.attws = b.take(L.attws_bytes / 4 + 64);
  L.total = b.off;
  return ACVAE_OK;
}
inline int step_attws_reset(float* sc, const StepLayout& L, hipStream_t st) {
  return L.attws_bytes > 0 ? zero(sc + L.attws, 256, st) : ACVAE_OK;
}
}

extern "C" int64_t acvae_step_scratch_bytes(int N, int S, int E, int H, int A, int V) {
  StepLayout L;
  return step_layout(N, S, E, H, A, V, L) == ACVAE_OK ? L.total * 4 : -1;
}

extern "C" int acvae_attn_precompute(const void* const* params, int which, const float* mem, float* encproj, int N,
                                     int S, int E, int H, int A, void* stream) {
  if (!params || !mem || !encproj || N <= 0 || S <= 0) return ACVAE_EINVAL;
  Ctx st{(hipStream_t)stream, nullptr};
  auto P = [&](int i) { return (const float*)params[i]; };
  if (which == 0) return gemm(mem, E, P(TP_DEC_ATT_W) + H, E + H, P(TP_DEC_ATT_B), encproj, A, N * S, A, E, 0, st);
  return gemm(mem, E, P(TP_P_ATT_W) + E, 2 * E, P(TP_P_ATT_B), encproj, E, N * S, E, E, 0, st);
}

namespace {
int prior_step(const void* const* params, const int64_t* word, const float* mem, const int64_t* mem_lens, const float* ep,
               const float* h_prev, const float* c_prev, const float* last_z, const float* eps, float* mean, float* logv,
               float* z, float* h_out, float* c_out, float* attw, float* sc, const StepLayout& L, int Nm, int Tq, int S,
               int E, int V, const Ctx& st) {
  auto P = [&](int i) { return (const float*)params[i]; };
  const int N = Nm * Tq, Hp = E;
  float* rnn = sc + L.rnn;
  float* q = sc + L.q;
  float* gates = sc + L.gates;
  float* ml = sc + L.ml;
  ACVAE_TRY(acvae::embed_gather(word, 1, P(TP_P_EMB), V, rnn, 3 * E, N, E, st));
  ACVAE_TRY(gemm(rnn, 3 * E, P(TP_P_ATT_W), 2 * E, nullptr, q, E, N, E, E, 0, st));
  ACVAE_TRY(acvae_attn_fwd(q, (long)Tq * E, E, ep, mem, mem_lens, P(TP_P_ATT_V), rnn + E, (long)Tq * 3 * E, 3 * E, attw,
                           (long)Tq * S, S, Nm, Tq, S, E, E, L.attws_bytes > 0 ? sc + L.attws : nullptr, L.attws_bytes, st, 0));
  ACVAE_TRY(acvae::copy_rows(rnn + 2 * E, 3 * E, last_z, E, N, E, st));
  ACVAE_TRY(gemm(rnn, 3 * E, P(TP_P_WIH), 3 * E, P(TP_P_BIH), gates, 4 * Hp, N, 4 * Hp, 3 * E, 0, st));
  ACVAE_TRY(gemm(h_prev, Hp, P(TP_P_WHH), Hp, P(TP_P_BHH), gates, 4 * Hp, N, 4 * Hp, Hp, 1, st));
  ACVAE_TRY(acvae::lstm_fwd(gates, 4 * Hp, c_prev, Hp, h_out, Hp, c_out, Hp, nullptr, 0, N, Hp, st));
  ACVAE_TRY(gemm(h_out, Hp, P(TP_P_ML_W), Hp, P(TP_P_ML_B), ml, 2 * E, N, 2 * E, Hp, 0, st));
  return acvae_reparam_fwd(ml, 2 * E, eps, E, mean, logv, z, E, nullptr, 0, N, E, st);
}

int decoder_step(const void* const* params, const int64_t* word, const float* h_prev, const float* mem,
                 const int64_t* mem_lens, const float* ed, const float* z, float* logits, float* h_out, float* attw,
                 float* rnn_input, float* sc, const StepLayout& L, int Nm, int Tq, int S, int E, int H, int A, int V,
                 const Ctx& st) {
  auto P = [&](int i) { return (const float*)params[i]; };
  const int N = Nm * Tq;
  float* q = sc + L.q;
  float* gi = sc + L.gates;
  float* gh = sc + L.gh;
  ACVAE_TRY(acvae::embed_gather(word, 1, P(TP_DEC_EMB), V, rnn_input, 3 * E, N, E, st));
  ACVAE_TRY(gemm(h_prev, H, P(TP_DEC_ATT_W), E + H, nullptr, q, A, N, A, H, 0, st));
  ACVAE_TRY(acvae_attn_fwd(q, (long)Tq * A, A, ed, mem, mem_lens, P(TP_DEC_ATT_V), rnn_input + E, (long)Tq * 3 * E, 3 * E,
                           attw, (long)Tq * S, S, Nm, Tq, S, A, E, L.attws_bytes > 0 ? sc + L.attws : nullptr, L.attws_bytes, st, 0));
  ACVAE_TRY(acvae::copy_rows(rnn_input + 2 * E, 3 * E, z, E, N, E, st));
  ACVAE_TRY(gemm(rnn_input, 3 * E, P(TP_DEC_WIH), 3 * E, P(TP_DEC_BIH), gi, 3 * H, N, 3 * H, 3 * E, 0, st));
  ACVAE_TRY(gemm(h_prev, H, P(TP_DEC_WHH), H, P(TP_DEC_BHH), gh, 3 * H, N, 3 * H, H, 0, st));
  ACVAE_TRY(acvae::gru_fwd(gi, 3 * H, gh, 3 * H, h_prev, H, h_out, H, nullptr, 0, nullptr, 0, nullptr, 0, nullptr, 0, N,
                           H, st));
  return gemm(h_out, H, P(TP_DEC_CLS_W), H, P(TP_DEC_CLS_B), logits, V, N, V, H, 0, st);
}
}

extern "C" int acvae_prior_step_fwd(const void* const* params, const int64_t* word, const float* mem,
                                    const int64_t* mem_lens, const float* encproj_p, const float* h_prev,
                                    const float* c_prev, const float* last_z, const float* eps, float* mean, float* logv,
                                    float* z, float* h_out, float* c_out, float* attw, void* scratch_v,
                                    int64_t scratch_bytes, int N, int S, int E, int V, void* stream) {
  StepLayout L;
  ACVAE_TRY(step_layout(N, S, E, E, E, V, L));
  if (!params || !word || !mem || !mem_lens || !h_prev || !c_prev || !last_z || !eps || !mean || !logv || !z ||
      !h_out || !c_out || !attw || !scratch_v)
    return ACVAE_EINVAL;
  if (scratch_bytes < L.total * 4) return ACVAE_EWORKSPACE;
  float* sc = (float*)scratch_v;
  Ctx st{(hipStream_t)stream, sc + L.skws};
  ACVAE_TRY(acvae_skinny_ws_reset(st.skws, st.s));
  ACVAE_TRY(step_attws_reset(sc, L, st.s));
  const float* ep = encproj_p;
  if (!ep) {
    ACVAE_TRY(acvae_attn_precompute(params, 1, mem, sc + L.encproj, N, S, E, E, E, stream));
    ep = sc + L.encproj;
  }
  return prior_step(params, word, mem, mem_lens, ep, h_prev, c_prev, last_z, eps, mean, logv, z, h_out, c_out, attw, sc,
                    L, N, 1, S, E, V, st);
}

extern "C" int acvae_decoder_step_fwd(const void* const* params, const int64_t* word, const float* h_prev,
                                      const float* mem, const int64_t* mem_lens, const float* encproj_d, const float* z,
                                      float* logits, float* h_out, float* attw, float* rnn_input, void* scratch_v,
                                      int64_t scratch_bytes, int N, int S, int E, int H, int A, int V, void* stream) {
  StepLayout L;
  ACVAE_TRY(step_layout(N, S, E, H, A, V, L));
  if (!params || !word || !h_prev || !mem || !mem_lens || !z || !logits || !h_out || !attw || !rnn_input || !scratch_v)
    return ACVAE_EINVAL;
  if (scratch_bytes < L.total * 4) return ACVAE_EWORKSPACE;
  float* sc = (float*)scratch_v;
  Ctx st{(hipStream_t)stream, sc + L.skws};
  ACVAE_TRY(acvae_skinny_ws_reset(st.skws, st.s));
  ACVAE_TRY(step_attws_reset(sc, L, st.s));
  const float* ed = encproj_d;
  if (!ed) {
    ACVAE_TRY(acvae_attn_precompute(params, 0, mem, sc + L.encproj, N, S, E, H, A, stream));
    ed = sc + L.encproj;
  }
  return decoder_step(params, word, h_prev, mem, mem_lens, ed, z, logits, h_out, attw, rnn_input, sc, L, N, 1, S, E, H,
                      A, V, st);
}

namespace {
struct BeamLayout { long step, encd, encp, h, hp, cp, lz, mean, logv, z, h2, hp2, cp2, attp, logits, rnn, lse, topk, scores,
                    attw, words, total; };
int beam_layout(int N, int beam, int T, int S, int E, int H, int A, int V, BeamLayout& L) {
  if (N <= 0 || beam <= 0 || T <= 0) return ACVAE_EINVAL;
  StepLayout sl;
  const long R = (long)N * beam;
  if (R > (1L << 20)) return ACVAE_EUNSUPPORTED;
  ACVAE_TRY(step_layout((int)R, S, E, H, A, V, sl));
  Bump b;
  L.step = b.take(sl.total);
  L.encd = b.take((long)N * S * A);
  L.encp = b.take((long)N * S * E);
  L.h = b.take(R * H); L.hp = b.take(R * E); L.cp = b.take(R * E); L.lz = b.take(R * E);
  L.mean = b.take(R * E); L.logv = b.take(R * E); L.z = b.take(R * E);
  L.h2 = b.take(R * H); L.hp2 = b.take(R * E); L.cp2 = b.take(R * E);
  L.attp = b.take(R * S);
  L.logits = b.take(R * V);
  L.rnn = b.take(R * 3 * E);
  L.lse = b.take(R);
  L.topk = b.take(R);
  L.scores = b.take(R * V);
  L.attw = b.take((long)T * R * S);
  L.words = b.take(2 * ((long)(3 * T + 1) * R));
  L.total = b.off;
  return ACVAE_OK;
}

struct GatherJob { const float* src; float* dst; int width; };
using GatherTable = acvae::JobTable<GatherJob, 4>;
__global__ __launch_bounds__(256) void beam_gather_kernel(GatherTable g, const int64_t* __restrict__ parent) {
  const GatherJob j = g.job[blockIdx.y];
  const long r = blockIdx.x, p = parent[r];
  for (int i = threadIdx.x; i < j.width; i += blockDim.x) j.dst[r * j.width + i] = j.src[p * j.width + i];
}

__global__ __launch_bounds__(256) void beam_trace_kernel(const int64_t* __restrict__ parent, const int64_t* __restrict__ word,
                                                         const float* __restrict__ attw, int64_t* __restrict__ seqs,
                                                         float* __restrict__ attw_out, long hist_stride, int R, int beam, int T,
                                                         int S) {
  const int n = blockIdx.x;
  long r = (long)n * beam;
  for (int t = T - 1; t >= 0; --t) {
    const long p = parent[t * hist_stride + r];
    if (threadIdx.x == 0) seqs[(long)n * T + t] = word[t * hist_stride + r];
    const float* w = attw + ((long)t * R + p) * S;
    for (int s = threadIdx.x; s < S; s += blockDim.x) attw_out[((long)n * S + s) * T + t] = w[s];
    r = p;
  }
}
__global__ void fill_words_kernel(int64_t* w, int64_t v, int n) {
  const int i = blockIdx.x * blockDim.x + threadIdx.x;
  if (i < n) w[i] = v;
}
}

extern "C" int64_t acvae_beam_search_scratch_bytes(int N, int beam, int max_length, int S, int E, int H, int A, int V) {
  BeamLayout L;
  return beam_layout(N, beam, max_length, S, E, H, A, V, L) == ACVAE_OK ? L.total * 4 : -1;
}

extern "C" int acvae_beam_search(const void* const* params, const float* mem, const int64_t* mem_lens, const float* eps,
                                 int64_t start_idx, int64_t* seqs, float* attw_out, void* scratch_v, int64_t scratch_bytes,
                                 int N, int beam, int max_length, int S, int E, int H, int A, int V, void* stream) {
  BeamLayout L;
  ACVAE_TRY(beam_layout(N, beam, max_length, S, E, H, A, V, L));
  if (!params || !mem || !mem_lens || !eps || !seqs || !attw_out || !scratch_v) return ACVAE_EINVAL;
  if (start_idx < 0 || start_idx >= V || beam > 64 || H != E) return ACVAE_EINVAL;
  if (scratch_bytes < L.total * 4) return ACVAE_EWORKSPACE;
  StepLayout SL;
  const int R = N * beam, T = max_length;
  ACVAE_TRY(step_layout(R, S, E, H, A, V, SL));
  float* sc = (float*)scratch_v;
  float* ssc = sc + L.step;
  Ctx st{(hipStream_t)stream, ssc + SL.skws};
  ACVAE_TRY(acvae_skinny_ws_reset(st.skws, st.s));
  ACVAE_TRY(step_attws_reset(ssc, SL, st.s));
  ACVAE_TRY(acvae_attn_precompute(params, 0, mem, sc + L.encd, N, S, E, H, A, stream));
  ACVAE_TRY(acvae_attn_precompute(params, 1, mem, sc + L.encp, N, S, E, E, E, stream));
  float *h = sc + L.h, *hp = sc + L.hp, *cp = sc + L.cp, *lz = sc + L.lz;
  float *h2 = sc + L.h2, *hp2 = sc + L.hp2, *cp2 = sc + L.cp2, *z = sc + L.z;
  float* topk = sc + L.topk;
  int64_t* word = (int64_t*)(sc + L.words);
  int64_t* hist = word + R;
  ACVAE_TRY(zero(h, (long)R * H, st));
  ACVAE_TRY(zero(hp, (long)R * E, st));
  ACVAE_TRY(zero(cp, (long)R * E, st));
  ACVAE_TRY(zero(lz, (long)R * E, st));
  ACVAE_TRY(zero(topk, R, st));
  hipLaunchKernelGGL(fill_words_kernel, dim3((R + 255) / 256), dim3(256), 0, st.s, word, start_idx, R);
  const int64_t* w_t = word;
  for (int t = 0; t < T; ++t) {
    float* attw_t = sc + L.attw + (long)t * R * S;
    int64_t* idx_t = hist + (long)t * 3 * R;
    int64_t* par_t = idx_t + R;
    int64_t* nxt_t = par_t + R;
    ACVAE_TRY(prior_step(params, w_t, mem, mem_lens, sc + L.encp, hp, cp, lz, eps + (long)t * R * E, sc + L.mean,
                         sc + L.logv, z, hp2, cp2, sc + L.attp, ssc, SL, N, beam, S, E, V, st));
    ACVAE_TRY(decoder_step(params, w_t, h, mem, mem_lens, sc + L.encd, z, sc + L.logits, h2, attw_t, sc + L.rnn, ssc, SL,
                           N, beam, S, E, H, A, V, st));
    ACVAE_TRY(acvae_row_logsoftmax_argmax(sc + L.logits, V, V, nullptr, nullptr, sc + L.lse, 1, 1, R, 1, V, stream));
    ACVAE_TRY(acvae_logprob_add(sc + L.logits, V, sc + L.lse, topk, sc + L.scores, R, V, stream));
    ACVAE_TRY(acvae_topk_flat_batched(sc + L.scores, (int64_t)beam * V, (int64_t)beam * V, beam, V, topk, idx_t, par_t,
                                      nxt_t, N, beam, stream));
    if (t + 1 < T) {
      GatherTable g;
      g.add({h2, h, H}); g.add({hp2, hp, E}); g.add({cp2, cp, E}); g.add({z, lz, E});
      hipLaunchKernelGGL(beam_gather_kernel, dim3(R, g.n), dim3(256), 0, st.s, g, par_t);
      w_t = nxt_t;
    }
  }
  hipLaunchKernelGGL(beam_trace_kernel, dim3(N), dim3(256), 0, st.s, hist + R, hist + 2 * R, sc + L.attw, seqs, attw_out,
                     3L * R, R, beam, T, S);
  ACVAE_LAUNCH_CHECK();
  return ACVAE_OK;
}
```

### acvae_amd/csrc/gemm.hip

```cpp
#include <cstdlib>
#include "mfma_tile.h"
#include "../../include/acvae_hip.h"
#include "conv.h"

namespace {
using namespace mfma;

template <int BN, bool VEC4>
__global__ __launch_bounds__(nt_threads<128>(), 2) void gemm_nt_kernel(const float* __restrict__ A, long lda,
                                                                     const float* __restrict__ B, long ldb,
                                                                     const float* __restrict__ bias,
                                                                     float* __restrict__ C, long ldc, int M, int N,
                                                                     int K, int accumulate) {
  __shared__ NtSmem<128, BN> sm;
  PlainLoader<VEC4, 4> al{A, lda, M, K};
  PlainLoader<VEC4, BN / 32> bl{B, ldb, N, K};
  PlainEpilogue ep{C, ldc, bias, accumulate};
  int bm, bn;
  xcd_tile(gridDim.x, gridDim.y, bm, bn);
  nt_block<128, BN>(al, bl, M, N, K, bm, bn, ep, sm);
}

template <int WM, int WN, bool VEC4>
__global__ __launch_bounds__(256, 2) void gemm_tn_kernel(const float* __restrict__ A, long lda,
                                                         const float* __restrict__ B, long ldb, float* __restrict__ C,
                                                         long ldc, int M, int N, int K, int k_per, int accumulate,
                                                         long slab_stride) {
  __shared__ TnSmem<WM, WN> sm;
  PlainKMajorLoader<VEC4> al{A, lda, M, K}, bl{B, ldb, N, K};
  const int kb = blockIdx.z * k_per;
  const int ke = min(K, kb + k_per);
  float* out = C + (long)blockIdx.z * slab_stride;
  tn_block<WM, WN>(al, bl, M, N, kb, ke, blockIdx.x, blockIdx.y, out, ldc, accumulate, sm);
}

__global__ void slab_reduce_kernel(const float* __restrict__ slab, long slab_stride, int nsplit, float* __restrict__ C,
                                   long ldc, int M, int N, int accumulate) {
  const long total = (long)M * N;
  for (long i = blockIdx.x * (long)blockDim.x + threadIdx.x; i < total; i += (long)gridDim.x * blockDim.x) {
    const int m = (int)(i / N), n = (int)(i % N);
    float acc = 0.f;
    for (int z = 0; z < nsplit; ++z) acc += slab[z * slab_stride + i];
    float* p = C + (long)m * ldc + n;
    *p = accumulate ? *p + acc : acc;
  }
}

template <int WM, int WN, bool VEC4>
__global__ __launch_bounds__(256, 2) void gemm_tn_fused_kernel(const float* __restrict__ A, long lda, const float* __restrict__ B,
                                                               long ldb, float* __restrict__ slab, float* __restrict__ C, long ldc,
                                                               int M, int N, int K, int k_per, int accumulate, long slab_stride,
                                                               unsigned* __restrict__ tickets) {
  __shared__ TnSmem<WM, WN> sm;
  __shared__ int s_last;
  PlainKMajorLoader<VEC4> al{A, lda, M, K}, bl{B, ldb, N, K};
  const int kb = blockIdx.z * k_per;
  const int ke = min(K, kb + k_per);
  tn_block<WM, WN, true>(al, bl, M, N, kb, ke, blockIdx.x, blockIdx.y, slab + (long)blockIdx.z * slab_stride, (long)N, 0, sm);
  asm volatile("s_waitcnt vmcnt(0)" ::: "memory");
  __syncthreads();
  if (threadIdx.x == 0) {
    unsigned* tk = tickets + blockIdx.y * gridDim.x + blockIdx.x;
    const unsigned t = __hip_atomic_fetch_add(tk, 1u, __ATOMIC_RELAXED, __HIP_MEMORY_SCOPE_AGENT);
    s_last = t == gridDim.z - 1 ? 1 : 0;
    if (s_last) __hip_atomic_store(tk, 0u, __ATOMIC_RELAXED, __HIP_MEMORY_SCOPE_AGENT);
  }
  __syncthreads();
  if (!s_last) return;
  constexpr int TM = WM * 64, TN = WN * 64;
  const int m0 = blockIdx.x * TM, n0 = blockIdx.y * TN;
  const int nsplit = gridDim.z;
  for (int i = threadIdx.x; i < TM * TN; i += 256) {
    const int m = m0 + i / TN, n = n0 + i % TN;
    if (m >= M || n >= N) continue;
    const long e = (long)m * N + n;
    float acc = 0.f;
    for (int z0 = 0; z0 < nsplit; z0 += 8) {
      float v[8];
#pragma unroll
      for (int u = 0; u < 8; ++u)
        v[u] = z0 + u < nsplit ? __hip_atomic_load(slab + (z0 + u) * slab_stride + e, __ATOMIC_RELAXED, __HIP_MEMORY_SCOPE_AGENT) : 0.f;
#pragma unroll
      for (int u = 0; u < 8; ++u)
        if (z0 + u < nsplit) acc += v[u];
    }
    float* p = C + (long)m * ldc + n;
    *p = accumulate ? *p + acc : acc;
  }
}

constexpr int SK_MAX_TILES = 1024;
template <bool VEC4>
__global__ __launch_bounds__(SK_THREADS) void gemm_skinny_kernel(const float* __restrict__ A1, long lda1,
                                                                 const float* __restrict__ B1, long ldb1, int K1,
                                                                 const float* __restrict__ A2, long lda2,
                                                                 const float* __restrict__ B2, long ldb2, int K2,
                                                                 const float* __restrict__ bias, float* __restrict__ C,
                                                                 long ldc, int M, int N, int accumulate,
                                                                 float* __restrict__ slabs, unsigned* __restrict__ cnt) {
  __shared__ float red[SK_WAVES][32][33];
  __shared__ int s_last;
  const int lane = threadIdx.x & 63, wave = threadIdx.x >> 6, li = lane & 31, lh = lane >> 5;
  const int n0 = blockIdx.x * 32, m0 = blockIdx.y * 32;
  const int S = gridDim.z, z = blockIdx.z;
  f32x16 acc;
#pragma unroll
  for (int r = 0; r < 16; ++r) acc[r] = 0.f;
  sk_accumulate<VEC4>(acc, A1, lda1, B1, ldb1, M, N, K1, m0, n0, z * SK_WAVES + wave, S * SK_WAVES, li, lh);
  if (A2) sk_accumulate<VEC4>(acc, A2, lda2, B2, ldb2, M, N, K2, m0, n0, z * SK_WAVES + wave, S * SK_WAVES, li, lh);
#pragma unroll
  for (int r = 0; r < 16; ++r) red[wave][(r & 3) + 8 * (r >> 2) + 4 * lh][li] = acc[r];
  __syncthreads();
  const int tile = blockIdx.y * gridDim.x + blockIdx.x;
  float* my = slabs + ((long)tile * S + z) * 1024;
  if (S > 1) {
    {
      const int e = threadIdx.x * 2;
      float v0 = 0.f, v1 = 0.f;
#pragma unroll
      for (int w = 0; w < SK_WAVES; ++w) { v0 += red[w][e >> 5][e & 31]; v1 += red[w][e >> 5][(e & 31) + 1]; }
      const unsigned long long bits = (unsigned long long)__float_as_uint(v0) | ((unsigned long long)__float_as_uint(v1) << 32);
      __hip_atomic_store(reinterpret_cast<unsigned long long*>(my + e), bits, __ATOMIC_RELAXED, __HIP_MEMORY_SCOPE_AGENT);
    }
    asm volatile("s_waitcnt vmcnt(0)" ::: "memory");
    __syncthreads();
    if (threadIdx.x == 0) {
      const unsigned t = __hip_atomic_fetch_add(&cnt[tile], 1u, __ATOMIC_RELAXED, __HIP_MEMORY_SCOPE_AGENT);
      const int last = (t == (unsigned)(S - 1));
      if (last) __hip_atomic_store(&cnt[tile], 0u, __ATOMIC_RELAXED, __HIP_MEMORY_SCOPE_AGENT);
      s_last = last;
    }
    __syncthreads();
    if (!s_last) return;
    const float* base = slabs + (long)tile * S * 1024;
    const int e = threadIdx.x * 2;
    float v0 = 0.f, v1 = 0.f;
    for (int q0 = 0; q0 < S; q0 += 8) {
      unsigned long long b[8];
#pragma unroll
      for (int u = 0; u < 8; ++u)
        b[u] = q0 + u < S ? __hip_atomic_load(reinterpret_cast<const unsigned long long*>(base + (long)(q0 + u) * 1024 + e),
                                              __ATOMIC_RELAXED, __HIP_MEMORY_SCOPE_AGENT) : 0ull;
#pragma unroll
      for (int u = 0; u < 8; ++u)
        if (q0 + u < S) { v0 += __uint_as_float((unsigned)b[u]); v1 += __uint_as_float((unsigned)(b[u] >> 32)); }
    }
    const int mm = e >> 5, m = m0 + mm;
#pragma unroll
    for (int k = 0; k < 2; ++k) {
      const int n = n0 + (e & 31) + k;
      if (m < M && n < N) {
        float v = k ? v1 : v0;
        if (bias) v += bias[n];
        float* p = C + (long)m * ldc + n;
        if (accumulate) v += *p;
        *p = v;
      }
    }
    return;
  }
  for (int e = threadIdx.x; e < 1024; e += SK_THREADS) {
    const int mm = e >> 5, nn = e & 31;
    const int m = m0 + mm, n = n0 + nn;
    if (m < M && n < N) {
      float v = 0.f;
#pragma unroll
      for (int w = 0; w < SK_WAVES; ++w) v += red[w][mm][nn];
      if (bias) v += bias[n];
      float* p = C + (long)m * ldc + n;
      if (accumulate) v += *p;
      *p = v;
    }
  }
}

__global__ void transpose_kernel(const float* __restrict__ in, long ld_in, float* __restrict__ out, long ld_out,
                                 int rows, int cols) {
  __shared__ float tile[32][33];
  const int c0 = blockIdx.x * 32, r0 = blockIdx.y * 32;
  for (int j = threadIdx.y; j < 32; j += 8) {
    const int r = r0 + j, c = c0 + threadIdx.x;
    tile[j][threadIdx.x] = (r < rows && c < cols) ? in[(long)r * ld_in + c] : 0.f;
  }
  __syncthreads();
  for (int j = threadIdx.y; j < 32; j += 8) {
    const int c = c0 + j, r = r0 + threadIdx.x;
    if (r < rows && c < cols) out[(long)c * ld_out + r] = tile[threadIdx.x][j];
  }
}

__global__ void transpose_batch_kernel(TransposeBatch b) {
  __shared__ float tile[32][33];
  const int m = b.find((int)blockIdx.x);
  const TransposeJob& job = b.job[m];
  const int t = blockIdx.x - b.start[m];
  const int tcols = (job.cols + 31) / 32;
  const int c0 = (t % tcols) * 32, r0 = (t / tcols) * 32;
  const float* in = job.in;
  float* out = job.out;
  const int rows = job.rows, cols = job.cols;
  for (int j = threadIdx.y; j < 32; j += 8) {
    const int r = r0 + j, c = c0 + threadIdx.x;
    tile[j][threadIdx.x] = (r < rows && c < cols) ? in[(long)r * job.ld_in + c] : 0.f;
  }
  __syncthreads();
  for (int j = threadIdx.y; j < 32; j += 8) {
    const int c = c0 + j, r = r0 + threadIdx.x;
    if (r < rows && c < cols) out[(long)c * job.ld_out + r] = tile[threadIdx.x][j];
  }
}

inline bool vec_ok(const float* p, int64_t ld, int k) { return aligned16(p) && (ld & 3) == 0 && (k & 3) == 0; }

}

int acvae_transpose_batch(TransposeBatch& b, hipStream_t st) {
  if (!b.ok()) return ACVAE_EINVAL;
  if (b.n <= 0) return ACVAE_OK;
  for (int m = 0; m < b.n; ++m) {
    const TransposeJob& j = b.job[m];
    if (!j.in || !j.out || j.rows <= 0 || j.cols <= 0) return ACVAE_EINVAL;
  }
  const int tiles = b.seal([](const TransposeJob& j) { return cdiv(j.cols, 32) * cdiv(j.rows, 32); });
  hipLaunchKernelGGL(transpose_batch_kernel, dim3(tiles), dim3(32, 8), 0, st, b);
  ACVAE_LAUNCH_CHECK();
  return ACVAE_OK;
}

long acvae_skinny_ws_floats() { return SK_MAX_TILES + (long)SK_MAX_TILES * 1024; }
long acvae_skinny_ticket_words() { return SK_MAX_TILES; }
int acvae_skinny_ws_reset(float* ws, hipStream_t st) {
  return hipMemsetAsync(ws, 0, SK_MAX_TILES * sizeof(unsigned), st) == hipSuccess ? ACVAE_OK : (int)hipGetLastError();
}

namespace {
struct SkProblem {
  const float* A; long lda;
  const float* B; long ldb;
  int K;
  const float* bias;
  float* C; long ldc;
  int N, accumulate;
};
template <bool VEC4>
__global__ __launch_bounds__(SK_THREADS) void gemm_skinny_pair_kernel(SkProblem p0, SkProblem p1, int nx0, int M) {
  __shared__ float red[SK_WAVES][32][33];
  const int lane = threadIdx.x & 63, wave = threadIdx.x >> 6, li = lane & 31, lh = lane >> 5;
  const bool second = (int)blockIdx.x >= nx0;
  const SkProblem& p = second ? p1 : p0;
  const int n0 = ((int)blockIdx.x - (second ? nx0 : 0)) * 32, m0 = blockIdx.y * 32;
  f32x16 acc;
#pragma unroll
  for (int r = 0; r < 16; ++r) acc[r] = 0.f;
  sk_accumulate<VEC4>(acc, p.A, p.lda, p.B, p.ldb, M, p.N, p.K, m0, n0, wave, SK_WAVES, li, lh);
#pragma unroll
  for (int r = 0; r < 16; ++r) red[wave][(r & 3) + 8 * (r >> 2) + 4 * lh][li] = acc[r];
  __syncthreads();
  for (int e = threadIdx.x; e < 1024; e += SK_THREADS) {
    const int mm = e >> 5, nn = e & 31;
    const int m = m0 + mm, n = n0 + nn;
    if (m < M && n < p.N) {
      float v = 0.f;
#pragma unroll
      for (int w = 0; w < SK_WAVES; ++w) v += red[w][mm][nn];
      if (p.bias) v += p.bias[n];
      float* o = p.C + (long)m * p.ldc + n;
      if (p.accumulate) v += *o;
      *o = v;
    }
  }
}
}

int acvae_gemm_nt_pair(const float* A0, int64_t lda0, const float* B0, int64_t ldb0, int K0, const float* bias0, float* C0,
                       int64_t ldc0, int N0, int acc0, const float* A1, int64_t lda1, const float* B1, int64_t ldb1, int K1,
                       const float* bias1, float* C1, int64_t ldc1, int N1, int acc1, int M, hipStream_t st) {
  if (!A0 || !B0 || !C0 || !A1 || !B1 || !C1 || M <= 0 || M > 64 || N0 <= 0 || N1 <= 0 || K0 <= 0 || K1 <= 0)
    return ACVAE_EINVAL;
  const bool vec = vec_ok(A0, lda0, K0) && vec_ok(B0, ldb0, K0) && vec_ok(A1, lda1, K1) && vec_ok(B1, ldb1, K1);
  const SkProblem p0{A0, lda0, B0, ldb0, K0, bias0, C0, ldc0, N0, acc0}, p1{A1, lda1, B1, ldb1, K1, bias1, C1, ldc1, N1, acc1};
  const int nx0 = cdiv(N0, 32);
  dim3 grid(nx0 + cdiv(N1, 32), cdiv(M, 32));
  if (vec) hipLaunchKernelGGL(gemm_skinny_pair_kernel<true>, grid, dim3(SK_THREADS), 0, st, p0, p1, nx0, M);
  else hipLaunchKernelGGL(gemm_skinny_pair_kernel<false>, grid, dim3(SK_THREADS), 0, st, p0, p1, nx0, M);
  ACVAE_LAUNCH_CHECK();
  return ACVAE_OK;
}

int acvae_gemm_nt_dual(const float* A1, int64_t lda1, const float* B1, int64_t ldb1, int K1, const float* A2,
                       int64_t lda2, const float* B2, int64_t ldb2, int K2, const float* bias, float* C, int64_t ldc,
                       int M, int N, int accumulate, hipStream_t st, float* skws) {
  if (!A1 || !B1 || !C || M <= 0 || N <= 0 || K1 <= 0) return ACVAE_EINVAL;
  if (A2 && (!B2 || K2 <= 0)) return ACVAE_EINVAL;
  bool vec = vec_ok(A1, lda1, K1) && vec_ok(B1, ldb1, K1);
  if (A2) vec = vec && vec_ok(A2, lda2, K2) && vec_ok(B2, ldb2, K2);
  const long big_blocks = (long)cdiv(M, 128) * cdiv(N, N <= 64 ? 64 : 128);
  if (M <= 64 || A2 || (big_blocks < 100 && M <= 4096)) {
    const int tiles = cdiv(N, 32) * cdiv(M, 32);
    int S = 1;
    const int Ktot = K1 + (A2 ? K2 : 0);
    static const bool splitk_on = !(getenv("ACVAE_SKINNY_SPLITK") && getenv("ACVAE_SKINNY_SPLITK")[0] == '0');
    if (skws && splitk_on && tiles <= 16 && Ktot >= 1024) {
      S = 128 / tiles;
      const int maxs = Ktot / 256;
      if (S > maxs) S = maxs;
      if (S > 8) S = 8;
      if (S < 1) S = 1;
      if ((long)tiles * S > SK_MAX_TILES) S = 1;
    }
    dim3 grid(cdiv(N, 32), cdiv(M, 32), S);
    unsigned* cnt = (unsigned*)skws;
    float* slabs = skws ? skws + SK_MAX_TILES : nullptr;
    if (vec)
      hipLaunchKernelGGL(gemm_skinny_kernel<true>, grid, dim3(SK_THREADS), 0, st, A1, lda1, B1, ldb1, K1, A2, lda2, B2,
                         ldb2, K2, bias, C, ldc, M, N, accumulate, slabs, cnt);
    else
      hipLaunchKernelGGL(gemm_skinny_kernel<false>, grid, dim3(SK_THREADS), 0, st, A1, lda1, B1, ldb1, K1, A2, lda2,
                         B2, ldb2, K2, bias, C, ldc, M, N, accumulate, slabs, cnt);
    ACVAE_LAUNCH_CHECK();
    return ACVAE_OK;
  }
  const bool bn64 = (N <= 64);
  dim3 grid(cdiv(M, 128), cdiv(N, bn64 ? 64 : 128));
#define LAUNCH_NT(BN_, V_)                                                                                     \
  hipLaunchKernelGGL((gemm_nt_kernel<BN_, V_>), grid, dim3(nt_threads<128>()), 0, st, A1, lda1, B1, ldb1, bias, C, ldc, M, \
                     N, K1, accumulate)
  if (bn64) { if (vec) LAUNCH_NT(64, true); else LAUNCH_NT(64, false); }
  else      { if (vec) LAUNCH_NT(128, true); else LAUNCH_NT(128, false); }
#undef LAUNCH_NT
  ACVAE_LAUNCH_CHECK();
  return ACVAE_OK;
}

extern "C" int acvae_gemm_nt(const float* A, int64_t lda, const float* B, int64_t ldb, const float* bias, float* C,
                             int64_t ldc, int M, int N, int K, int accumulate, void* stream) {
  return acvae_gemm_nt_dual(A, lda, B, ldb, K, nullptr, 0, nullptr, 0, 0, bias, C, ldc, M, N, accumulate,
                            (hipStream_t)stream, nullptr);
}

static int tn_splits(int M, int N, int K) {
  const long tiles = (long)cdiv(M, 128) * cdiv(N, 128);
  int s = (int)(256 / (tiles > 0 ? tiles : 1));
  const int maxs = cdiv(K, 4 * BKT);
  if (s > maxs) s = maxs;
  if (s < 1) s = 1;
  if (s > 256) s = 256;
  return s;
}

extern "C" int64_t acvae_gemm_tn_workspace_bytes(int M, int N, int K) {
  const int s = tn_splits(M, N, K);
  return s > 1 ? (int64_t)s * M * N * (int64_t)sizeof(float) : 0;
}

extern "C" int acvae_gemm_tn(const float* A, int64_t lda, const float* B, int64_t ldb, float* C, int64_t ldc, int M,
                             int N, int K, int accumulate, float* slab_ws, int64_t slab_ws_bytes, void* stream) {
  if (!A || !B || !C || M <= 0 || N <= 0 || K <= 0) return ACVAE_EINVAL;
  hipStream_t st = (hipStream_t)stream;
  int s = tn_splits(M, N, K);
  if (s > 1 && (!slab_ws || slab_ws_bytes < (int64_t)s * M * N * (int64_t)sizeof(float))) s = 1;
  int k_per = cdiv(cdiv(K, s), BKT) * BKT;
  s = cdiv(K, k_per);
  const bool vec = aligned16(A) && aligned16(B) && (lda & 3) == 0 && (ldb & 3) == 0 && (M & 3) == 0 && (N & 3) == 0;
  const bool narrow = (M <= 64);
  dim3 grid(cdiv(M, narrow ? 64 : 128), cdiv(N, narrow ? 256 : 128), s);
  float* out = s > 1 ? slab_ws : C;
  const long out_ld = s > 1 ? N : ldc;
  const long slab_stride = s > 1 ? (long)M * N : 0;
  const int acc_k = s > 1 ? 0 : accumulate;
#define LAUNCH_TN(WM_, WN_, V_)                                                                              \
  hipLaunchKernelGGL((gemm_tn_kernel<WM_, WN_, V_>), grid, dim3(256), 0, st, A, lda, B, ldb, out, out_ld, M, N, K, \
                     k_per, acc_k, slab_stride)
  if (narrow) { if (vec) LAUNCH_TN(1, 4, true); else LAUNCH_TN(1, 4, false); }
  else        { if (vec) LAUNCH_TN(2, 2, true); else LAUNCH_TN(2, 2, false); }
#undef LAUNCH_TN
  if (s > 1) {
    const long total = (long)M * N;
    hipLaunchKernelGGL(slab_reduce_kernel, dim3((int)((total + 255) / 256 > 2048 ? 2048 : (total + 255) / 256)),
                       dim3(256), 0, st, slab_ws, slab_stride, s, C, ldc, M, N, accumulate);
  }
  ACVAE_LAUNCH_CHECK();
  return ACVAE_OK;
}

int acvae_gemm_tn_fused(const float* A, int64_t lda, const float* B, int64_t ldb, float* C, int64_t ldc, int M, int N, int K,
                        int accumulate, float* ws, int64_t ws_bytes, hipStream_t st) {
  if (!A || !B || !C || M <= 0 || N <= 0 || K <= 0) return ACVAE_EINVAL;
  int s = tn_splits(M, N, K);
  const bool narrow = (M <= 64);
  dim3 grid(cdiv(M, narrow ? 64 : 128), cdiv(N, narrow ? 256 : 128), 1);
  if (s > 1 && (!ws || ws_bytes < (int64_t)TN_TICKETS * 4 + (int64_t)s * M * N * (int64_t)sizeof(float) ||
                (long)grid.x * grid.y > TN_TICKETS))
    return acvae_gemm_tn(A, lda, B, ldb, C, ldc, M, N, K, accumulate, nullptr, 0, st);
  int k_per = cdiv(cdiv(K, s), BKT) * BKT;
  s = cdiv(K, k_per);
  if (s <= 1) return acvae_gemm_tn(A, lda, B, ldb, C, ldc, M, N, K, accumulate, nullptr, 0, st);
  grid.z = s;
  const bool vec = aligned16(A) && aligned16(B) && (lda & 3) == 0 && (ldb & 3) == 0 && (M & 3) == 0 && (N & 3) == 0;
  unsigned* tickets = reinterpret_cast<unsigned*>(ws);
  float* slab = ws + TN_TICKETS;
#define LAUNCH_TNF(WM_, WN_, V_)                                                                                        \
  hipLaunchKernelGGL((gemm_tn_fused_kernel<WM_, WN_, V_>), grid, dim3(256), 0, st, A, lda, B, ldb, slab, C, ldc, M, N, K, k_per, \
                     accumulate, (long)M * N, tickets)
  if (narrow) { if (vec) LAUNCH_TNF(1, 4, true); else LAUNCH_TNF(1, 4, false); }
  else        { if (vec) LAUNCH_TNF(2, 2, true); else LAUNCH_TNF(2, 2, false); }
#undef LAUNCH_TNF
  ACVAE_LAUNCH_CHECK();
  return ACVAE_OK;
}

extern "C" int acvae_transpose(const float* in, int64_t ld_in, float* out, int64_t ld_out, int rows, int cols,
                               void* stream) {
  if (!in || !out || rows <= 0 || cols <= 0) return ACVAE_EINVAL;
  hipLaunchKernelGGL(transpose_kernel, dim3(cdiv(cols, 32), cdiv(rows, 32)), dim3(32, 8), 0, (hipStream_t)stream, in,
                     ld_in, out, ld_out, rows, cols);
  ACVAE_LAUNCH_CHECK();
  return ACVAE_OK;
}
```

### include/acvae_hip.h

```cpp
#ifndef ACVAE_HIP_H
#define ACVAE_HIP_H
#include <stdint.h>
#ifdef __cplusplus
extern "C" {
#endif

#define ACVAE_ABI_VERSION 3
int acvae_abi_version(void);

#define ACVAE_FLAG_NO_PERSIST 1
#define ACVAE_FLAG_DEFER_PARAM_GRADS 2
#define ACVAE_FLAG_NO_ATTN_SPLIT 4
#define ACVAE_FLAG_TEST_STALL 8

int acvae_persist_status_register(int device, void* status_words_host);

int acvae_gemm_nt(const float* A, int64_t lda, const float* B, int64_t ldb, const float* bias, float* C,
                  int64_t ldc, int M, int N, int K, int accumulate, void* stream);
int acvae_gemm_tn(const float* A, int64_t lda, const float* B, int64_t ldb, float* C, int64_t ldc, int M, int N,
                  int K, int accumulate, float* slab_ws, int64_t slab_ws_bytes, void* stream);
int64_t acvae_gemm_tn_workspace_bytes(int M, int N, int K);
int64_t acvae_colsum_workspace_bytes(int cols);
int acvae_colsum(const float* x, int rows, int cols, float* out, void* ws, int64_t ws_bytes, void* stream);
int acvae_transpose(const float* in, int64_t ld_in, float* out, int64_t ld_out, int rows, int cols, void* stream);

int64_t acvae_attn_fwd_workspace_bytes(int N, int Tq, int S, int A, int E);
int acvae_attn_fwd(const float* qproj, int64_t q_sn, int64_t q_sj, const float* encproj, const float* enc,
                   const int64_t* lens, const float* v, float* ctx, int64_t c_sn, int64_t c_sj, float* weights,
                   int64_t w_sn, int64_t w_sj, int N, int Tq, int S, int A, int E, void* ws, int64_t ws_bytes, void* stream,
                   int flags);
int acvae_tanh_att(const float* x, float* y, int64_t n, void* stream);
int64_t acvae_attn_bwd_workspace_bytes(int N, int Tq, int S, int A);
int acvae_attn_bwd(const float* dctx, int64_t dc_sn, int64_t dc_sj, const float* qproj, int64_t q_sn, int64_t q_sj,
                   const float* encproj, const float* enc, const int64_t* lens, const float* v,
                   const float* weights, int64_t w_sn, int64_t w_sj, float* dqproj, int64_t dq_sn, int64_t dq_sj,
                   float* dencproj, float* denc, float* dv_part, float* ws, int64_t ws_bytes, int N, int Tq, int S,
                   int A, int E, void* stream);

int acvae_reparam_fwd(const float* ml, int64_t ld_ml, const float* eps, int64_t ld_eps, float* mean, float* logv,
                      float* z, int64_t ld_out, float* z2, int64_t ld_z2, int rows, int E, void* stream);
int acvae_reparam_bwd(const float* dz, int64_t ld_dz, const float* dmean_ext, const float* dlog_ext, int64_t ld_ext,
                      const float* logv, int64_t ld_lv, const float* eps, int64_t ld_eps, float* dml, int64_t ld_dml,
                      int rows, int E, void* stream);

int64_t acvae_kl_partials(int64_t n_elem);
int acvae_gauss_kl_fwd(const float* mu1, const float* lv1, const float* mu2, const float* lv2, float* partials,
                       float* out_scalar, int64_t rows, int E, void* stream);
int acvae_gauss_kl_bwd(const float* mu1, const float* lv1, const float* mu2, const float* lv2, const float* grad_out,
                       float* dmu1, float* dlv1, float* dmu2, float* dlv2, int64_t rows, int E, void* stream);

int acvae_row_logsoftmax_argmax(const float* logits, int64_t ld_n, int64_t ld_t, int64_t* argmax, float* max_logprob,
                                float* lse, int64_t o_sn, int64_t o_st, int N, int T, int V, void* stream);
#define ACVAE_SAMPLE_GREEDY 0
#define ACVAE_SAMPLE_GUMBEL 1
#define ACVAE_SAMPLE_MULTINOMIAL 2
int acvae_sample_noise(float* noise, int64_t n, int method, uint64_t seed, void* stream);
int acvae_sample_next_word(const float* logits, int64_t ld_n, int64_t ld_t, const float* noise, int64_t nz_sn,
                           int64_t nz_st, int method, float temp, int64_t* w_out, float* logprob_out, int64_t o_sn,
                           int64_t o_st, int N, int T, int V, void* stream);
int acvae_ls_ce_fwd(const float* logits, int64_t ld_n, int64_t ld_t, const int64_t* targets, int64_t tg_sn,
                    const int64_t* lens1, const float* lse, float smoothing, int reduction, float* loss_rows,
                    float* out_scalar, int N, int T, int V, void* stream);
int acvae_ls_ce_bwd(const float* logits, int64_t ld_n, int64_t ld_t, const int64_t* targets, int64_t tg_sn,
                    const int64_t* lens1, const float* lse, float smoothing, int reduction, const float* grad_out,
                    const float* grad_rows, float* dlogits, int N, int T, int V, void* stream);
int acvae_mse_fwd(const float* a, const float* b, float* partials, float* out_scalar, int64_t n, void* stream);
int acvae_mse_bwd(const float* a, const float* b, const float* grad_out, float* da, float* db, int64_t n, void* stream);
int acvae_loss_combine_fwd(const float* ce, const float* kl, const float* mse, float w_kl, float w_mse, float* out, void* stream);
int acvae_loss_combine_bwd(const float* grad_out, float w_kl, float w_mse, float* g_ce, float* g_kl, float* g_mse, void* stream);

#define ACVAE_ENC_NPARAMS 55
#define ACVAE_ARCH_CNN10 0
#define ACVAE_ARCH_CNN14_16K 1
#define ACVAE_ENC_BF16 256
int acvae_encoder_nparams(int arch);
int acvae_encoder_out_dims(int arch, int T, int* S, int* C);
int64_t acvae_encoder_saved_bytes(int arch, int N, int T, int F);
int64_t acvae_encoder_scratch_bytes(int arch, int N, int T, int F);
int acvae_encoder_fwd(const void* const* params, const float* feats, float* audio_embeds, float* pooled,
                      void* saved, int64_t saved_bytes, void* scratch, int64_t scratch_bytes, int arch, int N, int T,
                      int F, int training, float p_block, float p_fc, uint64_t seed, const uint8_t* const* masks,
                      void* stream);
int acvae_encoder_bwd(const void* const* params, void* const* grads, const float* feats,
                      const float* d_audio_embeds, void* saved, int64_t saved_bytes, void* scratch,
                      int64_t scratch_bytes, int arch, int N, int T, int F, int training, float p_block, uint64_t seed,
                      const uint8_t* const* masks, void* stream);
int acvae_encoder_relu_mask(const void* saved, int64_t saved_bytes, int arch, int N, int T, int F, int site,
                            uint8_t* mask_nchw, void* stream);
int acvae_encoder_bwd_hooked(const void* const* params, void* const* grads, const float* feats,
                             const float* d_audio_embeds, void* saved, int64_t saved_bytes, void* scratch,
                             int64_t scratch_bytes, int arch, int N, int T, int F, int training, float p_block,
                             uint64_t seed, const uint8_t* const* masks, void* stream, void* block_done, void* user);

int64_t acvae_conv3x3_workspace_bytes(int N, int H, int W, int Cin, int Cout);
int acvae_conv3x3_fwd(const float* X, const float* W_oihw, const float* in_scale, const float* in_shift, float* Y,
                      const float* gamma, const float* beta, float* running_mean, float* running_var,
                      int64_t* num_batches_tracked, int training, float* bn_out, void* ws, int64_t ws_bytes, int N, int H,
                      int W, int Cin, int Cout, void* stream);
int acvae_conv3x3_dgrad(const float* dY, const float* W_oihw, float* dX, void* ws, int64_t ws_bytes, int N, int H, int W,
                        int Cin, int Cout, void* stream);
int acvae_conv3x3_wgrad(const float* dY, const float* X, const float* in_scale, const float* in_shift, float* dW_oihw,
                        void* ws, int64_t ws_bytes, int N, int H, int W, int Cin, int Cout, void* stream);
int acvae_conv1_first_bwd(const float* x, const float* bn0, const float* W1_oihw, const float* dY, float* dW1,
                          float* dgamma0, float* dbeta0, void* ws, int64_t ws_bytes, int N, int T, int F, void* stream);
int acvae_conv3x3_fwd_wino(const float* X, const float* W_oihw, const float* in_scale, const float* in_shift, float* Y,
                           const float* gamma, const float* beta, float* running_mean, float* running_var,
                           int64_t* num_batches_tracked, int training, float* bn_out, void* ws, int64_t ws_bytes, int N,
                           int H, int W, int Cin, int Cout, void* stream);
int acvae_conv3x3_dgrad_wino(const float* dY, const float* W_oihw, float* dX, void* ws, int64_t ws_bytes, int N, int H,
                             int W, int Cin, int Cout, void* stream);
int acvae_conv3x3_dgrad_bnred_wino(const float* dY, const float* W_oihw, float* dX, const float* Yprev, const float* bn_prev,
                                   float* sum_g, float* sum_gy, void* ws, int64_t ws_bytes, int N, int H, int W, int Cin,
                                   int Cout, void* stream);
int acvae_conv3x3_wgrad_wino(const float* dY, const float* X, const float* in_scale, const float* in_shift, float* dW_oihw,
                             void* ws, int64_t ws_bytes, int N, int H, int W, int Cin, int Cout, void* stream);
int acvae_conv3x3_fwd_bf16(const void* X, const float* W_oihw, const float* in_scale, const float* in_shift, void* Y,
                           const float* gamma, const float* beta, float* running_mean, float* running_var,
                           int64_t* num_batches_tracked, int training, float* bn_out, void* ws, int64_t ws_bytes, int N,
                           int H, int W, int Cin, int Cout, void* stream);
int acvae_conv3x3_dgrad_bf16(const void* dY, const float* W_oihw, void* dX, void* ws, int64_t ws_bytes, int N, int H, int W,
                             int Cin, int Cout, void* stream);
int acvae_conv3x3_wgrad_bf16(const void* dY, const void* X, const float* in_scale, const float* in_shift, float* dW_oihw,
                             void* ws, int64_t ws_bytes, int N, int H, int W, int Cin, int Cout, void* stream);
int64_t acvae_bn_workspace_bytes(int N, int H, int W, int C);
int acvae_bn_mel_fwd(const float* x, const float* gamma, const float* beta, float* running_mean, float* running_var,
                     int64_t* num_batches_tracked, int training, float* bn_out, void* ws, int64_t ws_bytes, int64_t rows,
                     int F, void* stream);
int acvae_bn_relu_pool_fwd(const float* Y, const float* bn, float* P, int N, int H, int W, int C, int pool, float p_drop,
                           uint64_t seed, int site, const uint8_t* keep_mask, void* stream);
int acvae_bn_relu_bwd(const float* Y, const float* dO, int upstream, const float* bn, float* dgamma, float* dbeta,
                      float* dY, void* ws, int64_t ws_bytes, int N, int H, int W, int C, int training, float p_drop,
                      uint64_t seed, int site, const uint8_t* keep_mask, void* stream);

int64_t acvae_rnn_workspace_bytes(int N, int Tc, int I, int H);
int acvae_gru_step(const float* x, const float* h, const float* w_ih, const float* w_hh, const float* b_ih,
                   const float* b_hh, float* h_out, void* ws, int64_t ws_bytes, int N, int I, int H, void* stream);
int acvae_lstm_step(const float* x, const float* h, const float* c, const float* w_ih, const float* w_hh,
                    const float* b_ih, const float* b_hh, float* h_out, float* c_out, void* ws, int64_t ws_bytes, int N,
                    int I, int H, void* stream);
int acvae_bigru_seq(const float* X, const int64_t* lens, const void* const* w, float* hidden, void* ws, int64_t ws_bytes,
                    int N, int Tc, int E, int H, void* stream);

#define ACVAE_TEXT_NPARAMS 35

int64_t acvae_posterior_saved_bytes(int N, int Tc, int E, int Hq, int V);
int64_t acvae_posterior_scratch_bytes(int N, int Tc, int E, int Hq, int V);
int acvae_posterior_fwd(const void* const* params, const int64_t* caps, int64_t ld_caps, const int64_t* lens1,
                        const float* eps_q, float* q_means, float* q_logs, float* q_z, float* q_means_utt,
                        void* saved, int64_t saved_bytes, void* scratch, int64_t scratch_bytes, int N, int Tc, int E,
                        int Hq, int V, void* stream, int flags);
int acvae_posterior_bwd(const void* const* params, void* const* grads, const int64_t* lens1, const float* eps_q,
                        const float* q_logs, const float* d_q_means, const float* d_q_logs, const float* d_q_z,
                        const float* d_q_means_utt, void* saved, int64_t saved_bytes, void* scratch,
                        int64_t scratch_bytes, int N, int Tc, int E, int Hq, int V, void* stream, int flags);


int64_t acvae_decode_saved_bytes(int N, int Tc, int S, int E, int H, int A, int V, int Eenc);
int64_t acvae_decode_scratch_bytes(int N, int Tc, int S, int E, int H, int A, int V, int Eenc);
int acvae_decode_fwd(const void* const* params, const float* mem_in, const int64_t* mem_lens, const int64_t* caps,
                     int64_t ld_caps, const int64_t* lens1, const float* q_z, const float* eps_p,
                     const int* ss_flags_host, const int* dis_flags_host, float* logits, float* outputs, int64_t* seqs,
                     float* sampled_logprobs, float* attn_w, float* p_means, float* p_logs, float* p_z,
                     float* p_means_utt, float* h_final, float* hp_final, float* cp_final, void* saved,
                     int64_t saved_bytes, void* scratch, int64_t scratch_bytes, int N, int Tc, int S, int E, int H,
                     int A, int V, int Eenc, int start_idx, int end_idx, void* stream, void* aux_stream, int flags);
int acvae_decode_fwd_sampled(const void* const* params, const float* mem_in, const int64_t* mem_lens,
                             const int64_t* caps, int64_t ld_caps, const int64_t* lens1, const float* q_z,
                             const float* eps_p, const int* ss_flags_host, const int* dis_flags_host, float* logits,
                             float* outputs, int64_t* seqs, float* sampled_logprobs, float* attn_w, float* p_means,
                             float* p_logs, float* p_z, float* p_means_utt, float* h_final, float* hp_final,
                             float* cp_final, void* saved, int64_t saved_bytes, void* scratch, int64_t scratch_bytes,
                             int N, int Tc, int S, int E, int H, int A, int V, int Eenc, int start_idx, int end_idx,
                             void* stream, void* aux_stream, int sample_method, float temp, const float* sample_noise,
                             const uint8_t* emb_keep, float emb_drop_p, int flags);
int acvae_decode_bwd_defers(const int* dis_flags_host, int Tc, void* stream, void* aux_stream, int flags);
int acvae_decode_bwd(const void* const* params, void* const* grads, const float* mem_in, const int64_t* mem_lens,
                     const int64_t* lens1, const float* eps_p, const int* dis_flags_host, const float* outputs,
                     const float* attn_w, const float* p_logs, const float* d_logits, const float* d_outputs_ext,
                     const float* d_p_means, const float* d_p_logs, const float* d_p_z, const float* d_p_means_utt,
                     float* d_mem_in, float* d_q_z, void* saved, int64_t saved_bytes, void* scratch,
                     int64_t scratch_bytes, int N, int Tc, int S, int E, int H, int A, int V, int Eenc, void* stream,
                     void* aux_stream, const uint8_t* emb_keep, float emb_drop_p, int flags);
int acvae_caps_to_long(const float* caps, int64_t* out, int64_t n, void* stream);

int64_t acvae_grad_norm_partials(void);
int acvae_grad_norm(const float* grads, int64_t n, float grad_scale, float* partials, float* out_norm, void* stream);
int acvae_adam_step(float* params, const float* grads, float* exp_avg, float* exp_avg_sq, int64_t n, float lr,
                    float beta1, float beta2, float eps, float weight_decay, int64_t step, float grad_scale,
                    float max_grad_norm, const float* total_norm, void* stream);
int acvae_adamw_step(float* params, const float* grads, float* exp_avg, float* exp_avg_sq, float* max_exp_avg_sq,
                     int64_t n, double lr, double beta1, double beta2, double eps, double weight_decay, int decoupled,
                     int amsgrad, int64_t step, float grad_scale, float max_grad_norm, const float* total_norm,
                     void* stream);
int acvae_sgd_step(float* params, const float* grads, float* momentum_buffer, int64_t n, double lr, double momentum,
                   double dampening, double weight_decay, int nesterov, int first, float grad_scale, float max_grad_norm,
                   const float* total_norm, void* stream);

int acvae_prof_enable(int enable);
int acvae_prof_pause(int paused);
int acvae_prof_read(int tag, double* total_ms_host, int64_t* launches_host);

int64_t acvae_step_scratch_bytes(int N, int S, int E, int H, int A, int V);
int acvae_attn_precompute(const void* const* params, int which, const float* mem, float* encproj, int N, int S, int E,
                          int H, int A, void* stream);
int acvae_prior_step_fwd(const void* const* params, const int64_t* word, const float* mem, const int64_t* mem_lens,
                         const float* encproj_p, const float* h_prev, const float* c_prev, const float* last_z,
                         const float* eps, float* mean, float* logv, float* z, float* h_out, float* c_out, float* attw,
                         void* scratch, int64_t scratch_bytes, int N, int S, int E, int V, void* stream);
int acvae_decoder_step_fwd(const void* const* params, const int64_t* word, const float* h_prev, const float* mem,
                           const int64_t* mem_lens, const float* encproj_d, const float* z, float* logits, float* h_out,
                           float* attw, float* rnn_input, void* scratch, int64_t scratch_bytes, int N, int S, int E,
                           int H, int A, int V, void* stream);
int acvae_logprob_add(const float* logits, int64_t ld, const float* lse, const float* prev, float* out, int N, int V,
                      void* stream);
int acvae_topk_flat(const float* x, int64_t n, int k, int V, float* vals, int64_t* idx, int64_t* row, int64_t* col,
                    void* stream);
int acvae_topk_flat_batched(const float* x, int64_t n, int64_t group_stride, int k, int V, float* vals, int64_t* idx,
                            int64_t* row, int64_t* col, int groups, int row_base, void* stream);
int64_t acvae_beam_search_scratch_bytes(int N, int beam, int max_length, int S, int E, int H, int A, int V);
int acvae_beam_search(const void* const* params, const float* mem, const int64_t* mem_lens, const float* eps,
                      int64_t start_idx, int64_t* seqs, float* attn_weights, void* scratch, int64_t scratch_bytes, int N,
                      int beam, int max_length, int S, int E, int H, int A, int V, void* stream);
int acvae_dbs_scores(const float* logits, int64_t ld, float temperature, const float* counts, float diversity_lambda,
                     const float* prev, float* out, int N, int V, int rows_per_count, void* stream);

#ifdef __cplusplus
}
#endif
#endif
```

Baseline: 2054.

## Batch weight-gradient TN GEMMs into a single grouped split-K kernel launch

Adds a grouped TN GEMM kernel that walks a table of jobs and handles each one's tiles and split-K slices inside one persistent grid, with per-job tickets and slab reduction. The decoder, posterior and prior backward passes now collect their weight-gradient GEMMs into groups and launch them together, and the dec and prior groups are merged when both run on the aux stream. The aim is to remove per-GEMM launch overhead and poor occupancy from many small skinny GEMMs. In exchange the workspace grows because each job needs its own slab, the colsum batch capacity is raised, and there is an optional fence build flag.

```diff
diff --git a/acvae_amd/build.py b/acvae_amd/build.py
--- a/acvae_amd/build.py
+++ b/acvae_amd/build.py
@@ -11,6 +11,8 @@
          "-ffp-contract=off"]
 if os.environ.get("ACVAE_EXACT_TANH") == "1":
     FLAGS.append("-DACVAE_EXACT_TANH")
+if os.environ.get("ACVAE_HANDOFF_FENCES") == "1":
+    FLAGS.append("-DACVAE_HANDOFF_FENCES")
 
 
 def sources():
diff --git a/acvae_amd/csrc/conv.h b/acvae_amd/csrc/conv.h
--- a/acvae_amd/csrc/conv.h
+++ b/acvae_amd/csrc/conv.h
@@ -71,7 +71,7 @@
 long colsum_ticket_words();
 int colsum2(const float* x, int P, int width, double* dpart, float* out, float* out2, int split, hipStream_t st);
 struct ColsumJob { const float* x; int P, width; float* out; float* out_b; int R; long d0; };
-using ColsumBatch = RangeTable<ColsumJob, 6, int>;
+using ColsumBatch = RangeTable<ColsumJob, 8, int>;
 int colsum_batch(ColsumBatch& b, double* dpart, long dpart_doubles, hipStream_t st);
 int conv1_first_blocks(int N, int T);
 template <class TY>
@@ -108,6 +108,14 @@
 constexpr int TN_TICKETS = 256;
 int acvae_gemm_tn_fused(const float* A, int64_t lda, const float* B, int64_t ldb, float* C, int64_t ldc, int M, int N, int K,
                         int accumulate, float* ws, int64_t ws_bytes, hipStream_t st);
+struct TnJob {
+  const float* A; long lda; const float* B; long ldb; float* C; long ldc; int M, N, K, accumulate;
+  int tm, tiles, s, k_per; float* slab; unsigned* tickets;
+};
+using TnGroup = acvae::RangeTable<TnJob, 16, int>;
+constexpr int TN_GROUP_TICKETS = 2048;
+long tn_group_slab_floats(int M, int N, int K);
+int acvae_gemm_tn_grouped(TnGroup& g, float* ws, int64_t ws_bytes, int max_blocks, hipStream_t st);
 long acvae_skinny_ws_floats();
 long acvae_skinny_ticket_words();
 int acvae_skinny_ws_reset(float* ws, hipStream_t st);
diff --git a/acvae_amd/csrc/decoder.hip b/acvae_amd/csrc/decoder.hip
--- a/acvae_amd/csrc/decoder.hip
+++ b/acvae_amd/csrc/decoder.hip
@@ -32,11 +32,22 @@
 struct TnWs { float* p; long bytes; };
 inline int gemm_tn(const float* A, long lda, const float* B, long ldb, float* C, long ldc, int M, int N, int K, TnWs ws,
                    hipStream_t st) {
-  return acvae_gemm_tn_fused(A, lda, B, ldb, C, ldc, M, N, K, 0, ws.p, ws.bytes, st);
+  const long off = TN_GROUP_TICKETS - TN_TICKETS;
+  return acvae_gemm_tn_fused(A, lda, B, ldb, C, ldc, M, N, K, 0, ws.p + off, ws.bytes - off * 4, st);
+}
+inline TnJob tn_job(const float* A, long lda, const float* B, long ldb, float* C, long ldc, int M, int N, int K) {
+  return TnJob{A, lda, B, ldb, C, ldc, M, N, K, 0, 0, 0, 0, 0, nullptr, nullptr};
+}
+inline int tn_group_blocks() {
+  static const int b = getenv("ACVAE_TN_GROUP_BLOCKS") ? atoi(getenv("ACVAE_TN_GROUP_BLOCKS")) : 0;
+  return b;
+}
+inline int gemm_tn_group(TnGroup& g, TnWs ws, hipStream_t st) {
+  return acvae_gemm_tn_grouped(g, ws.p, ws.bytes, tn_group_blocks(), st);
 }
 inline void zb_skinny(acvae::ZeroBatch& zb, float* skws) { zb.add(skws, acvae_skinny_ticket_words()); }
 inline void zb_colsum(acvae::ZeroBatch& zb, double* dpart) { zb.add(dpart, acvae::colsum_ticket_words()); }
-inline void zb_tn(acvae::ZeroBatch& zb, TnWs ws) { zb.add(ws.p, TN_TICKETS); }
+inline void zb_tn(acvae::ZeroBatch& zb, TnWs ws) { zb.add(ws.p, TN_GROUP_TICKETS); }
 inline int transp(const float* in, long ld_in, float* out, long ld_out, int rows, int cols, hipStream_t st) {
   return acvae_transpose(in, ld_in, out, ld_out, rows, cols, st);
 }
@@ -66,7 +77,7 @@
   int begin() const { return on() ? edge(main_s, aux) : ACVAE_OK; }
   int join() const { return on() ? edge(aux, main_s) : ACVAE_OK; }
 };
-inline long tn_ws_floats(int M, int N, int K) { return acvae_gemm_tn_workspace_bytes(M, N, K) / 4 + 64 + TN_TICKETS; }
+inline long tn_ws_floats(int M, int N, int K) { return acvae_gemm_tn_workspace_bytes(M, N, K) / 4 + 64 + TN_GROUP_TICKETS; }
 
 enum {
   TP_DEC_EMB, TP_DEC_WIH, TP_DEC_WHH, TP_DEC_BIH, TP_DEC_BHH, TP_DEC_CLS_W, TP_DEC_CLS_B, TP_DEC_ATT_V, TP_DEC_ATT_W,
@@ -108,11 +119,9 @@
   L.wt_ih0 = c.take((long)3 * Hq * E); L.wt_ih1 = c.take((long)3 * Hq * E); L.wt_ml = c.take((long)2 * E * 2 * Hq);
   L.pq_hbuf = c.take((long)4 * N * Hq);
   L.pq_cnt = c.take(acvae::posterior_persist_counter_words(Tc));
-  long tn = tn_ws_floats(2 * E, 2 * Hq, (int)R);
-  long t2 = tn_ws_floats(3 * Hq, E, (int)R); if (t2 > tn) tn = t2;
-  t2 = tn_ws_floats(3 * Hq, Hq, (int)R); if (t2 > tn) tn = t2;
-  L.tn_floats = tn;
-  L.tn = c.take(tn);
+  L.tn_floats = TN_GROUP_TICKETS + tn_group_slab_floats(2 * E, 2 * Hq, (int)R) +
+                2 * (tn_group_slab_floats(3 * Hq, E, (int)R) + tn_group_slab_floats(3 * Hq, Hq, (int)R));
+  L.tn = c.take(L.tn_floats);
   L.dpart_doubles = 4 * acvae::colsum_scratch_doubles(2 * E > 3 * Hq ? 2 * E : 3 * Hq);
   L.dpart = c.take(2 * L.dpart_doubles);
   L.skws = c.take(acvae_skinny_ws_floats());
@@ -130,7 +139,7 @@
       dlz_b, drnn, dz_dec, dqp, dmem, dhid, words_c, tn, dpart, attws, pd_cnt_b, pd_dqd, scratch_bwd;
   long dencproj_p, dvpart_p, dmem_p, drnn_p, tn_p, dpart_p, attws_p;
   long attws_bytes;
-  long tn_floats, tn_p_floats, dpart_doubles;
+  long tn_floats, tn_p_floats, dpart_doubles, dpart_p_doubles;
 };
 int dec_layout(int N, int Tc, int S, int E, int H, int A, int V, int Eenc, DecLayout& L) {
   if (N <= 0 || Tc <= 0 || S <= 0 || E <= 0 || H <= 0 || A <= 0 || V <= 1 || Eenc <= 0) return ACVAE_EINVAL;
@@ -173,13 +182,15 @@
   L.dc_b = b.take((long)N * Hp); L.dlz_a = b.take((long)N * E); L.dlz_b = b.take((long)N * E);
   L.drnn = b.take(R * 3 * E); L.dz_dec = b.take(R * E); L.dqp = b.take(R * E);
   L.dmem = b.take((long)N * S * E); L.dhid = b.take((long)N * H); L.words_c = b.take(R * 2);
-  long tn = 0;
-  auto mx = [&](int M, int Nn, int K) { const long t = tn_ws_floats(M, Nn, K); if (t > tn) tn = t; };
-  mx(V, H, (int)R); mx(3 * H, 3 * E, (int)R); mx(3 * H, H, (int)R); mx(A, H, (int)R); mx(A, E, N * S); mx(E, E, N * S);
-  mx(4 * Hp, 3 * E, (int)R); mx(4 * Hp, Hp, (int)R); mx(2 * E, Hp, (int)R); mx(E, E, (int)R); mx(2 * E, H, N);
-  mx(E, Eenc, N * S);
-  L.tn_floats = tn;
-  L.tn = b.take(tn);
+  const long g_heads = tn_group_slab_floats(V, H, (int)R) + tn_group_slab_floats(2 * E, H, N);
+  const long g_dec = tn_group_slab_floats(3 * H, 3 * E, (int)R) + tn_group_slab_floats(3 * H, H, (int)R) +
+                     tn_group_slab_floats(A, H, (int)R) + tn_group_slab_floats(A, E, N * S);
+  const long g_prior = tn_group_slab_floats(2 * E, Hp, (int)R) + tn_group_slab_floats(4 * Hp, 3 * E, (int)R) +
+                       tn_group_slab_floats(4 * Hp, Hp, (int)R) + tn_group_slab_floats(E, E, (int)R) +
+                       tn_group_slab_floats(E, E, N * S);
+  auto mx = [](long a, long b) { return a > b ? a : b; };
+  L.tn_floats = mx(TN_GROUP_TICKETS + mx(g_heads, g_dec), tn_ws_floats(E, Eenc, N * S));
+  L.tn = b.take(L.tn_floats);
   {
     int w = V; if (4 * Hp > w) w = 4 * Hp; if (3 * H > w) w = 3 * H; if (2 * E > w) w = 2 * E; if (A > w) w = A;
     L.dpart_doubles = acvae::colsum_scratch_doubles(w);
@@ -190,12 +201,10 @@
   L.attws_p = b.take(L.attws_bytes / 4 + 64);
   L.dencproj_p = b.take((long)N * S * E); L.dvpart_p = b.take((long)N * E); L.dmem_p = b.take((long)N * S * E);
   L.drnn_p = b.take(R * 3 * E);
-  L.tn_p_floats = L.tn_floats;
+  L.tn_p_floats = TN_GROUP_TICKETS + mx(g_heads, g_dec + g_prior);
   L.tn_p = b.take(L.tn_p_floats);
-  {
-    int w = V; if (4 * Hp > w) w = 4 * Hp; if (3 * H > w) w = 3 * H; if (2 * E > w) w = 2 * E; if (A > w) w = A;
-    L.dpart_p = b.take(2 * acvae::colsum_scratch_doubles(w));
-  }
+  L.dpart_p_doubles = mx(L.dpart_doubles, acvae::colsum_scratch_doubles(3 * H + 3 * H + A + A + 2 * E + 4 * Hp + E + E));
+  L.dpart_p = b.take(2 * L.dpart_p_doubles);
   L.pd_cnt_b = b.take(acvae::decode_persist_bwd_counter_words(Tc));
   L.pd_part = b.take(acvae::decode_persist_bwd_part_floats(N, E, H));
   L.pd_dqd = b.take(S > 64 && S <= 192 ? (long)acvae::decode_persist_bwd_rc_splits(S) * R * A : 0);
@@ -329,7 +338,8 @@
   if (d_q_means_utt)
     ACVAE_TRY(acvae::pool_bwd(d_q_means_utt, lens1, (const int*)(sv + L.argmax), dhid, (long)Tc * 2 * Hq, 2 * Hq, 1, N,
                               Tc, 2 * Hq, st));
-  ACVAE_TRY(gemm_tn(dml, 2 * E, hid, 2 * Hq, G(TP_Q_TML_W), 2 * Hq, 2 * E, 2 * Hq, R, tn, st));
+  TnGroup tg;
+  tg.add(tn_job(dml, 2 * E, hid, 2 * Hq, G(TP_Q_TML_W), 2 * Hq, 2 * E, 2 * Hq, R));
   acvae::ColsumBatch cb;
   cb.add({dml, R, 2 * E, G(TP_Q_TML_B)});
   float* dx = sc + L.dx;
@@ -367,12 +377,13 @@
         float* tmp = dh; dh = dh2; dh2 = tmp;
       }
     }
-    ACVAE_TRY(gemm_tn(dgi, 3 * Hq, X, E, G(TP_Q_WIH + o), E, 3 * Hq, E, R, tn, st));
+    tg.add(tn_job(dgi, 3 * Hq, X, E, G(TP_Q_WIH + o), E, 3 * Hq, E, R));
     cb.add({dgi, R, 3 * Hq, G(TP_Q_BIH + o)});
-    ACVAE_TRY(gemm_tn(dgh, 3 * Hq, hprev, Hq, G(TP_Q_WHH + o), Hq, 3 * Hq, Hq, R, tn, st));
+    tg.add(tn_job(dgh, 3 * Hq, hprev, Hq, G(TP_Q_WHH + o), Hq, 3 * Hq, Hq, R));
     cb.add({dgh, R, 3 * Hq, G(TP_Q_BHH + o)});
     ACVAE_TRY(gemm(dgi, 3 * Hq, wt_ih[dir], 3 * Hq, nullptr, dx, E, R, E, 3 * Hq, dir, st));
   }
+  ACVAE_TRY(gemm_tn_group(tg, tn, st));
   ACVAE_TRY(acvae::colsum_batch(cb, dpart, L.dpart_doubles, st));
   ACVAE_TRY(acvae::embed_scatter(words, dx, E, G(TP_Q_EMB), V, R, E, st));
   return ACVAE_OK;
@@ -727,20 +738,22 @@
   if (d_logits) ACVAE_TRY(gemm(d_logits, V, wt_cls, V, nullptr, d_out, H, R, H, V, 1, st));
   auto heads_params = [&](const Ctx& c, TnWs ws, double* dp) -> int {
     acvae::ColsumBatch cb;
+    TnGroup tg;
     if (d_p_means_utt) {
-      ACVAE_TRY(gemm_tn(d_p_means_utt, 2 * E, sv + L.pool_hid, H, G(TP_MLO_W), H, 2 * E, H, N, ws, c));
+      tg.add(tn_job(d_p_means_utt, 2 * E, sv + L.pool_hid, H, G(TP_MLO_W), H, 2 * E, H, N));
       cb.add({d_p_means_utt, N, 2 * E, G(TP_MLO_B)});
     } else {
       ACVAE_TRY(zero(G(TP_MLO_W), (long)2 * E * H, c));
       ACVAE_TRY(zero(G(TP_MLO_B), 2 * E, c));
     }
     if (d_logits) {
-      ACVAE_TRY(gemm_tn(d_logits, V, outputs, H, G(TP_DEC_CLS_W), H, V, H, R, ws, c));
+      tg.add(tn_job(d_logits, V, outputs, H, G(TP_DEC_CLS_W), H, V, H, R));
       cb.add({d_logits, R, V, G(TP_DEC_CLS_B)});
     } else {
       ACVAE_TRY(zero(G(TP_DEC_CLS_W), (long)V * H, c));
       ACVAE_TRY(zero(G(TP_DEC_CLS_B), V, c));
     }
+    ACVAE_TRY(gemm_tn_group(tg, ws, c));
     return acvae::colsum_batch(cb, dp, L.dpart_doubles, c);
   };
   static const bool heads_aux = !(getenv("ACVAE_HEADS_AUX") && atoi(getenv("ACVAE_HEADS_AUX")) == 0);
@@ -801,23 +814,29 @@
     }
     return ACVAE_OK;
   };
-  auto dec_params = [&](const Ctx& c, TnWs ws, double* dp, bool with_dz = true) -> int {
-    ACVAE_TRY(gemm_tn(dgi, 3 * H, rnn_d, 3 * E, G(TP_DEC_WIH), 3 * E, 3 * H, 3 * E, R, ws, c));
-    ACVAE_TRY(gemm_tn(dgh, 3 * H, hprev_d, H, G(TP_DEC_WHH), H, 3 * H, H, R, ws, c));
-    {
-      acvae::ColsumBatch cb;
-      cb.add({dgi, R, 3 * H, G(TP_DEC_BIH)}); cb.add({dgh, R, 3 * H, G(TP_DEC_BHH)});
-      cb.add({dencproj, N * S, A, G(TP_DEC_ATT_B)}); cb.add({dvpart, dv_rows, A, G(TP_DEC_ATT_V)});
-      ACVAE_TRY(acvae::colsum_batch(cb, dp, L.dpart_doubles, c));
-    }
-    ACVAE_TRY(gemm_tn(dqd, A, hprev_d, H, G(TP_DEC_ATT_W), E + H, A, H, R, ws, c));
-    ACVAE_TRY(gemm_tn(dencproj, A, mem, E, G(TP_DEC_ATT_W) + H, E + H, A, E, N * S, ws, c));
+  auto dec_tn = [&](TnGroup& tg, acvae::ColsumBatch& cb) {
+    tg.add(tn_job(dgi, 3 * H, rnn_d, 3 * E, G(TP_DEC_WIH), 3 * E, 3 * H, 3 * E, R));
+    tg.add(tn_job(dgh, 3 * H, hprev_d, H, G(TP_DEC_WHH), H, 3 * H, H, R));
+    tg.add(tn_job(dqd, A, hprev_d, H, G(TP_DEC_ATT_W), E + H, A, H, R));
+    tg.add(tn_job(dencproj, A, mem, E, G(TP_DEC_ATT_W) + H, E + H, A, E, N * S));
+    cb.add({dgi, R, 3 * H, G(TP_DEC_BIH)}); cb.add({dgh, R, 3 * H, G(TP_DEC_BHH)});
+    cb.add({dencproj, N * S, A, G(TP_DEC_ATT_B)}); cb.add({dvpart, dv_rows, A, G(TP_DEC_ATT_V)});
+  };
+  auto dec_rest = [&](const Ctx& c, bool with_dz) -> int {
     ACVAE_TRY(gemm(dgi, 3 * H, wt_dih, 3 * H, nullptr, drnn, E, R, E, 3 * H, 0, c));
     if (emb_keep)
       ACVAE_TRY(acvae::dropout_rows(drnn, (long)Tc * E, E, emb_keep, E, (long)N * E, emb_drop_p < 1.f ? 1.f / (1.f - emb_drop_p) : 0.f, N, Tc, E, c));
     if (with_dz) ACVAE_TRY(dec_dz(c));
     ACVAE_TRY(acvae::embed_scatter(words_c, drnn, E, G(TP_DEC_EMB), V, R, E, c));
     return ACVAE_OK;
+  };
+  auto dec_params = [&](const Ctx& c, TnWs ws, double* dp) -> int {
+    TnGroup tg;
+    acvae::ColsumBatch cb;
+    dec_tn(tg, cb);
+    ACVAE_TRY(gemm_tn_group(tg, ws, c));
+    ACVAE_TRY(acvae::colsum_batch(cb, dp, L.dpart_doubles, c));
+    return dec_rest(c, true);
   };
 
   float* dgates = sc + L.dgates;
@@ -878,20 +897,26 @@
                              dmem_p, dvpart_p, sc + L.attws_p, L.attws_bytes, N, Tc, S, E, E, sp));
     return gemm(dencproj_p, E, wt_patt + (long)E * E, E, nullptr, dmem_p, E, N * S, E, E, 1, sp);
   };
+  auto prior_tn = [&](TnGroup& tg, acvae::ColsumBatch& cb) {
+    tg.add(tn_job(dml_all, 2 * E, hp_all, Hp, G(TP_P_ML_W), Hp, 2 * E, Hp, R));
+    tg.add(tn_job(dgates, 4 * Hp, rnn_p, 3 * E, G(TP_P_WIH), 3 * E, 4 * Hp, 3 * E, R));
+    tg.add(tn_job(dgates, 4 * Hp, hpprev, Hp, G(TP_P_WHH), Hp, 4 * Hp, Hp, R));
+    tg.add(tn_job(dqp, E, rnn_p, 3 * E, G(TP_P_ATT_W), 2 * E, E, E, R));
+    tg.add(tn_job(dencproj_p, E, mem, E, G(TP_P_ATT_W) + E, 2 * E, E, E, N * S));
+    cb.add({dml_all, R, 2 * E, G(TP_P_ML_B)}); cb.add({dgates, R, 4 * Hp, G(TP_P_BIH), G(TP_P_BHH)});
+    cb.add({dencproj_p, N * S, E, G(TP_P_ATT_B)}); cb.add({dvpart_p, N, E, G(TP_P_ATT_V)});
+  };
+  auto prior_rest = [&]() -> int {
+    ACVAE_TRY(gemm(dqp, E, wt_patt, E, nullptr, drnn_p, 3 * E, R, E, E, 1, sp));
+    return acvae::embed_scatter(words_c, drnn_p, 3 * E, G(TP_P_EMB), V, R, E, sp);
+  };
   auto prior_params = [&]() -> int {
-    ACVAE_TRY(gemm_tn(dml_all, 2 * E, hp_all, Hp, G(TP_P_ML_W), Hp, 2 * E, Hp, R, tn_p, sp));
-    ACVAE_TRY(gemm_tn(dgates, 4 * Hp, rnn_p, 3 * E, G(TP_P_WIH), 3 * E, 4 * Hp, 3 * E, R, tn_p, sp));
-    ACVAE_TRY(gemm_tn(dgates, 4 * Hp, hpprev, Hp, G(TP_P_WHH), Hp, 4 * Hp, Hp, R, tn_p, sp));
-    {
-      acvae::ColsumBatch cb;
-      cb.add({dml_all, R, 2 * E, G(TP_P_ML_B)}); cb.add({dgates, R, 4 * Hp, G(TP_P_BIH), G(TP_P_BHH)});
-      cb.add({dencproj_p, N * S, E, G(TP_P_ATT_B)}); cb.add({dvpart_p, N, E, G(TP_P_ATT_V)});
-      ACVAE_TRY(acvae::colsum_batch(cb, dpart_p, L.dpart_doubles, sp));
-    }
-    ACVAE_TRY(gemm(dqp, E, wt_patt, E, nullptr, drnn_p, 3 * E, R, E, E, 1, sp));
-    ACVAE_TRY(gemm_tn(dqp, E, rnn_p, 3 * E, G(TP_P_ATT_W), 2 * E, E, E, R, tn_p, sp));
-    ACVAE_TRY(gemm_tn(dencproj_p, E, mem, E, G(TP_P_ATT_W) + E, 2 * E, E, E, N * S, tn_p, sp));
-    return acvae::embed_scatter(words_c, drnn_p, 3 * E, G(TP_P_EMB), V, R, E, sp);
+    TnGroup tg;
+    acvae::ColsumBatch cb;
+    prior_tn(tg, cb);
+    ACVAE_TRY(gemm_tn_group(tg, tn_p, sp));
+    ACVAE_TRY(acvae::colsum_batch(cb, dpart_p, L.dpart_p_doubles, sp));
+    return prior_rest();
   };
   if (prior_feeds_decoder) {
     ACVAE_TRY(dec_begin());
@@ -953,8 +978,14 @@
     ACVAE_TRY(dec_dz(st));
     ACVAE_TRY(Fork::edge(st.s, sp.s));
     if (!heads_on_aux) ACVAE_TRY(heads_params(sp, tn_p, dpart_p));
-    ACVAE_TRY(dec_params(sp, tn_p, dpart_p, false));
-    ACVAE_TRY(prior_params());
+    TnGroup tg;
+    acvae::ColsumBatch cb;
+    dec_tn(tg, cb);
+    prior_tn(tg, cb);
+    ACVAE_TRY(gemm_tn_group(tg, tn_p, sp));
+    ACVAE_TRY(acvae::colsum_batch(cb, dpart_p, L.dpart_p_doubles, sp));
+    ACVAE_TRY(dec_rest(sp, false));
+    ACVAE_TRY(prior_rest());
   }
   return ACVAE_OK;
 }
diff --git a/acvae_amd/csrc/gemm.hip b/acvae_amd/csrc/gemm.hip
--- a/acvae_amd/csrc/gemm.hip
+++ b/acvae_amd/csrc/gemm.hip
@@ -46,6 +46,46 @@
   }
 }
 
+__device__ __forceinline__ bool tn_ticket(unsigned* tk, int nsplit, int& s_last) {
+  __syncthreads();
+  if (threadIdx.x == 0) {
+#ifdef ACVAE_HANDOFF_FENCES
+    __builtin_amdgcn_fence(__ATOMIC_RELEASE, "agent");
+#endif
+    const unsigned t = __hip_atomic_fetch_add(tk, 1u, __ATOMIC_RELAXED, __HIP_MEMORY_SCOPE_AGENT);
+    s_last = t == (unsigned)nsplit - 1 ? 1 : 0;
+    if (s_last) __hip_atomic_store(tk, 0u, __ATOMIC_RELAXED, __HIP_MEMORY_SCOPE_AGENT);
+  }
+  __syncthreads();
+#ifdef ACVAE_HANDOFF_FENCES
+  if (s_last) __builtin_amdgcn_fence(__ATOMIC_ACQUIRE, "agent");
+#endif
+  return s_last != 0;
+}
+
+template <int TM, int TN>
+__device__ __forceinline__ void tn_slab_sum(const float* slab, long slab_stride, int nsplit, float* C, long ldc, int M, int N,
+                                            int bm, int bn, int accumulate) {
+  const int m0 = bm * TM, n0 = bn * TN;
+  for (int i = threadIdx.x; i < TM * TN; i += 256) {
+    const int m = m0 + i / TN, n = n0 + i % TN;
+    if (m >= M || n >= N) continue;
+    const long e = (long)m * N + n;
+    float acc = 0.f;
+    for (int z0 = 0; z0 < nsplit; z0 += 8) {
+      float v[8];
+#pragma unroll
+      for (int u = 0; u < 8; ++u)
+        v[u] = z0 + u < nsplit ? __hip_atomic_load(slab + (z0 + u) * slab_stride + e, __ATOMIC_RELAXED, __HIP_MEMORY_SCOPE_AGENT) : 0.f;
+#pragma unroll
+      for (int u = 0; u < 8; ++u)
+        if (z0 + u < nsplit) acc += v[u];
+    }
+    float* p = C + (long)m * ldc + n;
+    *p = accumulate ? *p + acc : acc;
+  }
+}
+
 template <int WM, int WN, bool VEC4>
 __global__ __launch_bounds__(256, 2) void gemm_tn_fused_kernel(const float* __restrict__ A, long lda, const float* __restrict__ B,
                                                                long ldb, float* __restrict__ slab, float* __restrict__ C, long ldc,
@@ -58,34 +98,32 @@
   const int ke = min(K, kb + k_per);
   tn_block<WM, WN, true>(al, bl, M, N, kb, ke, blockIdx.x, blockIdx.y, slab + (long)blockIdx.z * slab_stride, (long)N, 0, sm);
   asm volatile("s_waitcnt vmcnt(0)" ::: "memory");
-  __syncthreads();
-  if (threadIdx.x == 0) {
-    unsigned* tk = tickets + blockIdx.y * gridDim.x + blockIdx.x;
-    const unsigned t = __hip_atomic_fetch_add(tk, 1u, __ATOMIC_RELAXED, __HIP_MEMORY_SCOPE_AGENT);
-    s_last = t == gridDim.z - 1 ? 1 : 0;
-    if (s_last) __hip_atomic_store(tk, 0u, __ATOMIC_RELAXED, __HIP_MEMORY_SCOPE_AGENT);
-  }
-  __syncthreads();
-  if (!s_last) return;
-  constexpr int TM = WM * 64, TN = WN * 64;
-  const int m0 = blockIdx.x * TM, n0 = blockIdx.y * TN;
-  const int nsplit = gridDim.z;
-  for (int i = threadIdx.x; i < TM * TN; i += 256) {
-    const int m = m0 + i / TN, n = n0 + i % TN;
-    if (m >= M || n >= N) continue;
-    const long e = (long)m * N + n;
-    float acc = 0.f;
-    for (int z0 = 0; z0 < nsplit; z0 += 8) {
-      float v[8];
-#pragma unroll
-      for (int u = 0; u < 8; ++u)
-        v[u] = z0 + u < nsplit ? __hip_atomic_load(slab + (z0 + u) * slab_stride + e, __ATOMIC_RELAXED, __HIP_MEMORY_SCOPE_AGENT) : 0.f;
-#pragma unroll
-      for (int u = 0; u < 8; ++u)
-        if (z0 + u < nsplit) acc += v[u];
-    }
-    float* p = C + (long)m * ldc + n;
-    *p = accumulate ? *p + acc : acc;
+  if (!tn_ticket(tickets + blockIdx.y * gridDim.x + blockIdx.x, gridDim.z, s_last)) return;
+  tn_slab_sum<WM * 64, WN * 64>(slab, slab_stride, gridDim.z, C, ldc, M, N, blockIdx.x, blockIdx.y, accumulate);
+}
+
+__global__ __launch_bounds__(256, 2) void gemm_tn_grouped_kernel(TnGroup g) {
+  __shared__ TnSmem<2, 2> sm;
+  __shared__ int s_last;
+  const int total = g.start[g.n];
+  for (int item = blockIdx.x; item < total; item += gridDim.x) {
+    const int l = g.find(item);
+    const TnJob& j = g.job[l];
+    const int r = item - g.start[l];
+    const int t = r % j.tiles, z = r / j.tiles;
+    const int bm = t % j.tm, bn = t / j.tm;
+    PlainKMajorLoader<true> al{j.A, j.lda, j.M, j.K}, bl{j.B, j.ldb, j.N, j.K};
+    const int kb = z * j.k_per;
+    const int ke = min(j.K, kb + j.k_per);
+    if (j.s == 1) {
+      tn_block<2, 2>(al, bl, j.M, j.N, kb, ke, bm, bn, j.C, j.ldc, j.accumulate, sm);
+      continue;
+    }
+    const long slab_stride = (long)j.M * j.N;
+    tn_block<2, 2, true>(al, bl, j.M, j.N, kb, ke, bm, bn, j.slab + (long)z * slab_stride, (long)j.N, 0, sm);
+    asm volatile("s_waitcnt vmcnt(0)" ::: "memory");
+    if (!tn_ticket(j.tickets + t, j.s, s_last)) continue;
+    tn_slab_sum<128, 128>(j.slab, slab_stride, j.s, j.C, j.ldc, j.M, j.N, bm, bn, j.accumulate);
   }
 }
 
@@ -409,6 +447,89 @@
   return ACVAE_OK;
 }
 
+long tn_group_slab_floats(int M, int N, int K) {
+  const int s = tn_splits(M, N, K);
+  return s > 1 ? ((long)s * M * N + 63) & ~63L : 0;
+}
+
+int acvae_gemm_tn_grouped(TnGroup& g, float* ws, int64_t ws_bytes, int max_blocks, hipStream_t st) {
+  if (!g.ok()) return ACVAE_EINVAL;
+  if (g.n <= 0) return ACVAE_OK;
+  if (!ws || ws_bytes < (int64_t)TN_GROUP_TICKETS * 4) return ACVAE_EINVAL;
+  for (int l = 0; l < g.n; ++l) {
+    const TnJob& j = g.job[l];
+    if (!j.A || !j.B || !j.C || j.M <= 0 || j.N <= 0 || j.K <= 0) return ACVAE_EINVAL;
+  }
+  TnGroup rest;
+  int n = 0;
+  long tk = 0, slab = TN_GROUP_TICKETS;
+  const long ws_floats = ws_bytes / 4;
+  for (int l = 0; l < g.n; ++l) {
+    TnJob j = g.job[l];
+    const bool vec = aligned16(j.A) && aligned16(j.B) && (j.lda & 3) == 0 && (j.ldb & 3) == 0 && (j.M & 3) == 0 && (j.N & 3) == 0;
+    if (j.M <= 64 || !vec) { rest.add(j); continue; }
+    j.tm = cdiv(j.M, 128);
+    j.tiles = j.tm * cdiv(j.N, 128);
+    j.s = tn_splits(j.M, j.N, j.K);
+    j.k_per = cdiv(cdiv(j.K, j.s), BKT) * BKT;
+    j.s = cdiv(j.K, j.k_per);
+    j.slab = nullptr; j.tickets = nullptr;
+    if (j.s > 1) {
+      if (j.tiles > TN_TICKETS || tk + j.tiles > TN_GROUP_TICKETS) return ACVAE_EWORKSPACE;
+      j.tickets = reinterpret_cast<unsigned*>(ws) + tk;
+      tk += j.tiles;
+      const long need = tn_group_slab_floats(j.M, j.N, j.K);
+      if (slab + need > ws_floats) return ACVAE_EWORKSPACE;
+      j.slab = ws + slab;
+      slab += need;
+    }
+    int at = n++;
+    for (; at > 0 && g.job[at - 1].k_per < j.k_per; --at) g.job[at] = g.job[at - 1];
+    g.job[at] = j;
+  }
+  g.n = n;
+  if (n > 0) {
+    const int total = g.seal([](const TnJob& j) { return j.tiles * j.s; });
+    const int grid = max_blocks > 0 && total > max_blocks ? max_blocks : total;
+    hipLaunchKernelGGL(gemm_tn_grouped_kernel, dim3(grid), dim3(256), 0, st, g);
+    ACVAE_LAUNCH_CHECK();
+  }
+  for (int l = 0; l < rest.n; ++l) {
+    const TnJob& j = rest.job[l];
+    ACVAE_TRY(acvae_gemm_tn_fused(j.A, j.lda, j.B, j.ldb, j.C, j.ldc, j.M, j.N, j.K, j.accumulate,
+                                  ws + (TN_GROUP_TICKETS - TN_TICKETS), ws_bytes - (int64_t)(TN_GROUP_TICKETS - TN_TICKETS) * 4, st));
+  }
+  return ACVAE_OK;
+}
+
+extern "C" int64_t acvae_gemm_tn_fused_workspace_bytes(int M, int N, int K) {
+  return (int64_t)TN_TICKETS * 4 + acvae_gemm_tn_workspace_bytes(M, N, K);
+}
+extern "C" int acvae_gemm_tn_fused_c(const float* A, int64_t lda, const float* B, int64_t ldb, float* C, int64_t ldc, int M, int N,
+                                     int K, int accumulate, float* ws, int64_t ws_bytes, void* stream) {
+  return acvae_gemm_tn_fused(A, lda, B, ldb, C, ldc, M, N, K, accumulate, ws, ws_bytes, (hipStream_t)stream);
+}
+extern "C" int64_t acvae_gemm_tn_grouped_workspace_bytes(int njobs, const int* M, const int* N, const int* K) {
+  if (njobs < 0 || (njobs > 0 && (!M || !N || !K))) return -1;
+  long f = TN_GROUP_TICKETS;
+  for (int l = 0; l < njobs; ++l) {
+    if (M[l] <= 0 || N[l] <= 0 || K[l] <= 0) return -1;
+    f += tn_group_slab_floats(M[l], N[l], K[l]);
+  }
+  return (int64_t)f * 4;
+}
+extern "C" int acvae_gemm_tn_grouped_c(int njobs, const void* const* A, const int64_t* lda, const void* const* B,
+                                       const int64_t* ldb, void* const* C, const int64_t* ldc, const int* M, const int* N,
+                                       const int* K, const int* accumulate, float* ws, int64_t ws_bytes, int max_blocks,
+                                       void* stream) {
+  if (njobs < 0 || (njobs > 0 && (!A || !lda || !B || !ldb || !C || !ldc || !M || !N || !K || !accumulate))) return ACVAE_EINVAL;
+  TnGroup g;
+  for (int l = 0; l < njobs; ++l)
+    g.add({(const float*)A[l], lda[l], (const float*)B[l], ldb[l], (float*)C[l], ldc[l], M[l], N[l], K[l], accumulate[l],
+           0, 0, 0, 0, nullptr, nullptr});
+  return acvae_gemm_tn_grouped(g, ws, ws_bytes, max_blocks, (hipStream_t)stream);
+}
+
 extern "C" int acvae_transpose(const float* in, int64_t ld_in, float* out, int64_t ld_out, int rows, int cols,
                                void* stream) {
   if (!in || !out || rows <= 0 || cols <= 0) return ACVAE_EINVAL;
diff --git a/include/acvae_hip.h b/include/acvae_hip.h
--- a/include/acvae_hip.h
+++ b/include/acvae_hip.h
@@ -20,6 +20,13 @@
 int acvae_gemm_tn(const float* A, int64_t lda, const float* B, int64_t ldb, float* C, int64_t ldc, int M, int N,
                   int K, int accumulate, float* slab_ws, int64_t slab_ws_bytes, void* stream);
 int64_t acvae_gemm_tn_workspace_bytes(int M, int N, int K);
+int64_t acvae_gemm_tn_fused_workspace_bytes(int M, int N, int K);
+int acvae_gemm_tn_fused_c(const float* A, int64_t lda, const float* B, int64_t ldb, float* C, int64_t ldc, int M, int N,
+                          int K, int accumulate, float* ws, int64_t ws_bytes, void* stream);
+int64_t acvae_gemm_tn_grouped_workspace_bytes(int njobs, const int* M, const int* N, const int* K);
+int acvae_gemm_tn_grouped_c(int njobs, const void* const* A, const int64_t* lda, const void* const* B, const int64_t* ldb,
+                            void* const* C, const int64_t* ldc, const int* M, const int* N, const int* K,
+                            const int* accumulate, float* ws, int64_t ws_bytes, int max_blocks, void* stream);
 int64_t acvae_colsum_workspace_bytes(int cols);
 int acvae_colsum(const float* x, int rows, int cols, float* out, void* ws, int64_t ws_bytes, void* stream);
 int acvae_transpose(const float* in, int64_t ld_in, float* out, int64_t ld_out, int rows, int cols, void* stream);
```

Measured after the change: 2064 (median of 6 runs). No clear change (+0.5%).
